# AliBahri94/GM3D

Measured on AMD Instinct MI355X. Metric: point-clouds/sec pretrain step (N=1024,G=64), higher is better.
Workload: dtype bf16

## Files before the change

### gm3d_amd/_capi.py

```python
import ctypes
import os

_HERE = os.path.dirname(os.path.abspath(__file__))
LIB_PATH = os.environ.get("GM3D_HIP_LIB") or os.path.join(_HERE, "lib", "libgm3d_hip.so")

GM3D_OK, GM3D_EINVAL, GM3D_EUNSUPPORTED, GM3D_ELAUNCH = 0, -1, -2, -3
GM3D_F32, GM3D_BF16 = 0, 1

_vp, _i, _f = ctypes.c_void_p, ctypes.c_int, ctypes.c_float

SIGNATURES = {
    "gm3d_abi_version": [],
    "gm3d_strerror": [_i],
    "gm3d_fps": [_vp, _i, _i, _i, _vp, _vp, _vp],
    "gm3d_gather_points": [_vp, _vp, _i, _i, _i, _i, _vp, _vp],
    "gm3d_gather_points_grad": [_vp, _vp, _i, _i, _i, _i, _vp, _vp],
    "gm3d_knn": [_vp, _vp, _i, _i, _i, _i, _vp, _vp, _vp],
    "gm3d_knn_group": [_vp, _vp, _i, _i, _i, _i, _vp, _vp, _vp, _vp],
    "gm3d_chamfer_fwd": [_vp, _vp, _i, _i, _i, _vp, _vp, _vp, _vp, _vp],
    "gm3d_chamfer_bwd": [_vp, _vp, _vp, _vp, _vp, _vp, _i, _i, _i, _vp, _vp, _vp],
    "gm3d_patch_chamfer_loss_fwd": [_vp, ctypes.c_longlong, _vp, _vp, ctypes.c_longlong, _i, _i, _i, _vp, _vp, _vp, _vp, _i, _vp],
    "gm3d_patch_chamfer_loss_bwd": [_vp, ctypes.c_longlong, _vp, _vp, ctypes.c_longlong, _vp, _vp, _vp, _i, _i, _i, _vp, _i, _vp],
    "gm3d_attention_fwd": [_vp, _vp, _vp, _i, _i, _i, _f, _i, _vp],
    "gm3d_attention_qkv_fwd": [_vp, _vp, _vp, _vp, _vp, _i, _i, _i, _i, _f, _i, _vp],
    "gm3d_attention_bwd": [_vp, _vp, _vp, _vp, _vp, _i, _i, _i, _f, _i, _vp],
    "gm3d_ln_plain_partial_rows": [_i],
    "gm3d_ln_plain_fwd": [_vp, _vp, _vp, _f, _vp, _vp, _vp, _i, _i, _i, _vp],
    "gm3d_ln_plain_bwd": [_vp, _vp, _vp, _vp, _vp, _vp, _vp, _i, _i, _i, _vp],
    "gm3d_residual_ln_fwd": [_vp, _vp, _vp, _vp, _i, _vp, _vp, _vp, _f, _vp, _vp, _vp, _vp, _i, _i, _i, _vp],
    "gm3d_residual_ln_bwd": [_vp, _vp, _vp, _vp, _vp, _vp, _vp, _i, _vp, _vp, _vp, _vp, _vp, _i, _i, _i, _vp],
    "gm3d_ln_partial_rows": [_i],
    "gm3d_colsum_finish": [_vp, _i, _i, _i, _vp, _i, _vp],
    "gm3d_colsum_finish_batched": [_vp, _i, ctypes.c_longlong, _i, _i, _i, _vp, _i, _vp],
    "gm3d_bias_gelu_fwd": [_vp, _vp, _vp, _i, _i, _i, _vp],
    "gm3d_bias_gelu_bwd": [_vp, _vp, _vp, _vp, _vp, _i, _i, _i, _vp],
    "gm3d_gelu_partial_rows": [_i],
    "gm3d_embed_partial_rows": [_i, _i, _i],
    "gm3d_moments3": [_vp, _i, _vp, _vp],
    "gm3d_pn_layer1_fwd": [_vp, _vp, _vp, _vp, _i, _i, _i, _vp],
    "gm3d_group_max_fwd": [_vp, _vp, _vp, _vp, _i, _i, _i, _i, _vp],
    "gm3d_group_max_bwd": [_vp, _vp, _vp, _i, _i, _i, _i, _vp],
    "gm3d_bn_bcast_stats": [_vp, _vp, _i, _i, _i, _vp, _i, _vp],
    "gm3d_bn_bcast_apply_relu": [_vp, _vp, _vp, _vp, _vp, _i, _i, _i, _f, _i, _vp],
    "gm3d_bn_bcast_bwd_stats": [_vp, _vp, _vp, _vp, _vp, _vp, _vp, _i, _i, _i, _vp, _f, _i, _vp],
    "gm3d_bn_bcast_bwd_apply": [_vp, _vp, _vp, _vp, _vp, _vp, _vp, _vp, _vp, _vp, _vp, _i, _i, _i, _f, _i, _vp],
    "gm3d_head_fold": [_vp, _vp, _i, _i, _vp, _vp, _vp, _i, _vp],
    "gm3d_head_rowdot": [_vp, _vp, _vp, _i, _i, _vp, _i, _vp],
    "gm3d_head_fold_bwd": [_vp, _vp, _i, _i, _i, _vp, _vp, _vp],
    "gm3d_head_outer": [_vp, _vp, _i, _i, _vp, _i, _vp],
    "gm3d_scale_translate": [_vp, _vp, _f, _f, _f, _i, _i, _vp],
    "gm3d_group_select_maps": [_vp, _i, _i, _i, _i, _vp, _vp, _vp],
    "gm3d_bn_bcast_apply_relu_sel": [_vp, _vp, _vp, _vp, _vp, _vp, _i, _i, _i, _f, _i, _vp],
    "gm3d_bn_bcast_bwd_stats_sel": [_vp, _vp, _vp, _vp, _vp, _vp, _vp, _vp, _i, _i, _i, _vp, _f, _i, _vp],
    "gm3d_bn_bcast_bwd_apply_sel": [_vp, _vp, _vp, _vp, _vp, _vp, _vp, _vp, _vp, _vp, _vp, _vp, _i, _i, _i, _f, _i, _vp],
    "gm3d_lin3_gelu_fwd": [_vp, _vp, _vp, _vp, _i, _i, _i, _vp],
    "gm3d_lin3_gelu_bwd": [_vp, _vp, _vp, _vp, _i, _i, _vp, _i, _vp],
    "gm3d_lin3_finish": [_vp, _i, _i, _vp, _vp, _vp],
    "gm3d_rank_loss": [_vp, _vp, _i, _i, _vp, _vp, _vp],
    "gm3d_rank_loss_tail": [_vp, _i, _vp, _i, _i, _vp, _vp, _vp, _vp, _vp],
    "gm3d_rank_loss_tail_bwd": [_vp, _vp, _vp, _i, _i, _i, _vp, _vp],
    "gm3d_ema_counters": [_vp, _vp, _i, _f, _f, _vp],
    "gm3d_drop_path_scales": [_vp, _vp, _i, _i, _vp, _vp],
    "gm3d_pad_cols": [_vp, ctypes.c_longlong, _i, _i, _vp, _i, _i, _vp],
    "gm3d_patch_chamfer_loss_bwd_full": [_vp, ctypes.c_longlong, _vp, _vp, ctypes.c_longlong, _vp, _vp, _vp, _i, _i, _i, _i, _vp, _i, _vp],
    "gm3d_mask_select_b": [_vp, _vp, _i, _i, _i, _i, _vp, _vp, _vp, _vp, _i, _vp],
    "gm3d_pn1_bwd_finalize": [_vp, _vp, _vp, _vp, _vp, _vp, _vp, _vp, _i, _vp],
    "gm3d_gemm_tn_bf16": [_vp, _vp, _vp, _vp, _i, _i, _i, _i, _i, _i, _vp],
    "gm3d_gemm_tn_bf16_gelu": [_vp, _vp, _vp, _vp, _vp, _i, _i, _i, _i, _i, _i, _i, _vp],
    "gm3d_gemm_tn_bf16_pool": [_vp, _vp, _vp, _vp, _vp, _vp, _i, _i, _i, _i, _i, _i, _i, _i, _vp],
    "gm3d_gemm_tn_bf16_gelu_bwd": [_vp, _vp, _vp, _vp, _vp, _vp, _i, _i, _i, _i, _i, _i, _i, _vp],
    "gm3d_gemm_tn_bf16_res": [_vp, _vp, _vp, _vp, _vp, _i, _vp, _vp, _vp, _vp, _i, _i, _i, _i, _i, _i, _vp],
    "gm3d_gemm_tn_bf16_lna": [_vp, _vp, _vp, _vp, _f, _vp, _vp, _vp, _vp, _vp, _vp, _vp, _i, _i, _i, _i, _i, _i, _i, _vp],
    "gm3d_gemm_tile_rows": [_i],
    "gm3d_gemm_tn_bf16_ring": [_vp, _vp, _vp, _vp, _i, _i, _i, _i, _i, _i, _i, _vp],
    "gm3d_gemm_tn_bf16_ws": [_vp, _vp, _vp, _vp, _i, _i, _i, _i, _i, _i, _vp],
    "gm3d_gemm_tn_bf16_ws_pool": [_vp, _vp, _vp, _vp, _vp, _vp, _i, _i, _i, _i, _i, _i, _i, _i, _vp],
    "gm3d_gemm_ws_supported": [_i, _i, _i],
    "gm3d_gemm_tn_bf16_ws_poolg": [_vp, _vp, _vp, _vp, _vp, _vp, _i, _i, _i, _i, _i, _i, _i, _i, _i, _vp],
    "gm3d_gemm_nt_bf16_sum": [_vp, _vp, _vp, _vp, _vp, _i, _i, _i, _i, _i, _i, _i, ctypes.c_longlong, ctypes.c_longlong, ctypes.c_longlong, _i, _vp],
    "gm3d_gemm_nt_tiles": [_i, _i],
    "gm3d_gemm_nt_bf16_multi": [_i] + [_vp] * 14 + [_vp],
    "gm3d_gemm_tn_bf16_ws_bn_apply": [_vp, _vp, _vp, _vp, _vp, _f, _vp, _i, _i, _i, _i, _i, _i, _i, _vp],
    "gm3d_gemm_tn_bf16_ws_bn_stats": [_vp, _vp, _vp, _vp, _vp, _i, _i, _i, _i, _i, _i, _i, _vp],
    "gm3d_gemm_ws_stats_rows": [_i, _i, _i],
    "gm3d_gemm_tn_bf16_ws_bn_apply_g": [_vp, _vp, _vp, _vp, _vp, _f, _vp, _i, _i, _i, _i, _i, _i, _i, _i, _vp],
    "gm3d_gemm_tn_bf16_ws_bn_stats_g": [_vp, _vp, _vp, _vp, _vp, _i, _i, _i, _i, _i, _i, _i, _i, _vp],
    "gm3d_gemm_tn_bf16_ring96": [_vp, _vp, _vp, _vp, _i, _i, _i, _i, _i, _i, _i, _vp],
    "gm3d_gemm_tn_bf16_dma": [_vp, _vp, _vp, _vp, _i, _i, _i, _i, _i, _i, _i, _vp],
    "gm3d_gemm_tn_bf16_dma_gelu_bwd": [_vp, _vp, _vp, _vp, _vp, _vp, _i, _i, _i, _i, _i, _i, _i, _i, _vp],
    "gm3d_gemm_tn_bf16_dma_gelu": [_vp, _vp, _vp, _vp, _vp, _i, _i, _i, _i, _i, _i, _i, _i, _vp],
    "gm3d_transpose_bf16_batched": [_vp, _vp, _i, _i, _i, ctypes.c_longlong, _vp],
    "gm3d_transpose_bf16_multi": [_i, _vp, _vp, _vp, _vp, _vp, _vp, _vp],
    "gm3d_token_assemble_fwd": [_vp, _vp, _vp, _i, _i, _i, _i, _vp, _vp, _vp, _i, _vp],
    "gm3d_token_assemble_bwd": [_vp, _vp, _vp, _vp, _i, _i, _i, _i, _vp, _vp, _i, _vp],
    "gm3d_sum_few_rows": [_vp, _i, _i, ctypes.c_longlong, _vp, _vp],
    "gm3d_gemm_nt_bf16": [_vp, _vp, _vp, _i, _i, _i, _i, _i, _i, _i, ctypes.c_longlong, ctypes.c_longlong, ctypes.c_longlong, _i,
                          ctypes.c_longlong, _vp],
    "gm3d_gemm_nt_bf16_big": [_vp, _vp, _vp, _i, _i, _i, _i, _i, _i, _i, ctypes.c_longlong, ctypes.c_longlong, ctypes.c_longlong, _i,
                              ctypes.c_longlong, _vp],
    "gm3d_gemm_nt_splits": [_i, _i, _i, _i],
    "gm3d_radius_mask_bits": [_vp, _vp, _f, _i, _i, _vp, _vp],
    "gm3d_radius_mask_bits_m": [_vp, _vp, _i, _f, _i, _i, _vp, _vp],
    "gm3d_attention_masked_fwd": [_vp, _vp, _vp, _vp, _i, _i, _i, _i, _f, _i, _vp],
    "gm3d_attention_masked_bwd": [_vp, _vp, _vp, _vp, _vp, _vp, _i, _i, _i, _i, _f, _i, _vp],
    "gm3d_mask_select": [_vp, _vp, _i, _i, _i, _i, _vp, _vp, _vp, _i, _vp],
    "gm3d_bn_finalize": [_vp, ctypes.c_double, _vp, _vp, _f, _f, _vp, _vp, _vp, _vp, _vp, _vp, _vp, _i, _i, _vp],
    "gm3d_pn1_finalize": [_vp, ctypes.c_double, _vp, _vp, _vp, _vp, _f, _f, _vp, _vp, _vp, _vp, _vp, _vp, _vp, _vp, _vp, _i, _i, _vp],
    "gm3d_flat_partial_rows": [ctypes.c_longlong],
    "gm3d_adamw_ema_flat_step": [_vp, _vp, _vp, _vp, _vp, _vp, _vp, ctypes.c_longlong, ctypes.c_longlong, _vp, _f, _f, _f, _f,
                                 _vp, _f, _vp, _vp, _vp, _vp],
    "gm3d_adamw_ema_flat_step_lrd": [_vp, _vp, _vp, _vp, _vp, _vp, _vp, ctypes.c_longlong, ctypes.c_longlong, _vp, _vp, _f, _f,
                                     _f, _f, _vp, _f, _vp, _vp, _vp, _vp],
    "gm3d_group_scatter_add": [_vp, _vp, _vp, _i, _i, _i, _vp, _i, _vp],
    "gm3d_pn_layer1_bwd_stats": [_vp, _vp, _vp, _vp, _vp, _vp, _vp, _vp, _i, _i, _vp, _i, _vp],
    "gm3d_colsum_finish_f64": [_vp, _i, _i, _i, _vp, _vp],
    "gm3d_colsum_partial": [_vp, _i, _i, _vp, _i, _vp],
    "gm3d_gather_inverse": [_vp, _i, _i, _i, _vp, _vp, _vp],
    "gm3d_gather_rows_bwd": [_vp, _vp, _vp, _vp, _i, _i, _i, _i, _i, _vp],
    "gm3d_add_ln_fwd": [_vp, _vp, _vp, _vp, _i, _vp, _vp, _vp, _f, _vp, _vp, _vp, _vp, _i, _i, _i, _vp],
    "gm3d_add_ln_bwd": [_vp, _vp, _vp, _vp, _vp, _vp, _vp, _i, _vp, _vp, _vp, _i, _i, _i, _i, _vp],
    "gm3d_add_ln_bwd_acc": [_vp, _vp, _vp, _vp, _vp, _vp, _vp, _i, _vp, _vp, _vp, _i, _vp, _i, _i, _i, _i, _vp],
    "gm3d_partition_visible": [_vp, _i, _i, _i, _vp, _vp, _vp, _vp, _vp, _vp, _vp],
    "gm3d_select_rows": [_vp, _vp, _vp, _vp, _i, _i, _i, _i, _i, _vp],
    "gm3d_back_project": [_vp, _vp, _i, _i, _i, _i, _vp, _vp],
    "gm3d_interp3_fwd": [_vp, _vp, _vp, _vp, _vp, _i, _i, _i, _i, _i, _i, _vp],
    "gm3d_gather_rows_bwd_w": [_vp, _i, _i, _i, _vp, _vp, _vp, _vp, _i, _i, _i, _i, _i, _vp],
    "gm3d_where_rows": [_vp, _i, _vp, _vp, _i, _vp, ctypes.c_longlong, _i, _i, _vp],
    "gm3d_take_rows": [_vp, _vp, _vp, _i, _i, _i, _i, _i, _vp],
    "gm3d_colsum_partial_w": [_vp, _vp, _i, _i, _vp, _i, _vp],
    "gm3d_gemm_tn_bf16_dma_pool": [_vp, _vp, _vp, _vp, _vp, _vp, _i, _i, _i, _i, _i, _i, _i, _i, _i, _i, _vp],
    "gm3d_gemm_tn_bf16_dmaw": [_vp, _vp, _vp, _vp, _i, _i, _i, _i, _i, _i, _i, _i, _vp],
    "gm3d_vote_sample": [_vp, _vp, _vp, _vp, _vp, _i, _i, _i, _i, _i, _vp, _vp],
    "gm3d_cls_tail_vote": [_vp, _i, _i, _i, _i] + [_vp] * 14 + [_i, _f, _vp, _vp, _vp, _vp, _vp, _i, _vp],
    "gm3d_cls_tail_fwd": [_vp, _i, _i, _i, _i] + [_vp] * 10 + [_i] + [_vp] * 6 + [_f, _f, _i] + [_vp] * 8 + [_i, _vp],
    "gm3d_cls_tail_bwd": [_i, _i, _i, _i] + [_vp] * 7 + [_i, _i] + [_vp] * 21 + [_i, _vp],
    "gm3d_cls_tail_vote_pool": [_vp, _i, _i, _i, _i, _i] + [_vp] * 14 + [_i, _f, _vp, _vp, _vp, _vp, _vp, _vp, _i, _vp],
    "gm3d_svm_gram": [_vp, _i, _i, _vp, _vp],
    "gm3d_svm_smo": [_vp, _i, _i, _vp, ctypes.c_double, ctypes.c_double, ctypes.c_longlong, _vp, _vp, _vp, _vp, _vp],
    "gm3d_svm_weights": [_vp, _i, _i, _i, _vp, _vp, _vp, _vp],
    "gm3d_svm_predict": [_vp, _i, _i, _i, _vp, _vp, _vp, _vp, _vp, _vp],
}


class Gm3dError(RuntimeError):
    pass


def _load():
    if not os.path.exists(LIB_PATH):
        raise ImportError(
            "gm3d_amd: %s not found. Build it with `python -m gm3d_amd.build` "
            "(hipcc, --offload-arch=gfx950). There is no CPU fallback." % LIB_PATH)
    lib = ctypes.CDLL(LIB_PATH)
    for name, argtypes in SIGNATURES.items():
        fn = getattr(lib, name)
        fn.argtypes = argtypes
        fn.restype = ctypes.c_char_p if name == "gm3d_strerror" else ctypes.c_int
    return lib


lib = _load()


def check(rc, what):
    if rc != GM3D_OK:
        raise Gm3dError("%s failed: %s (code %d)" % (what, lib.gm3d_strerror(rc).decode(), rc))
```

### gm3d_amd/csrc/gemm_dma.hip

```cpp
#include "mfma.hpp"

namespace gm3d {

constexpr int DBK = 64;

template <int WMI, int EPI, int NJ>
__global__ __launch_bounds__(256, 2) void gemm_tn_dma_kernel(const bf16_t* __restrict__ A, const bf16_t* __restrict__ W,
                                                             const float* __restrict__ bias, bf16_t* __restrict__ C, int M, int N, int K,
                                                             int lda, int ldw, int ldc, int tiles_n, int total_tiles,
                                                             bf16_t* __restrict__ G, int ldg, const bf16_t* __restrict__ Fpre,
                                                             int ldfp, float* __restrict__ colpart, uint8_t* __restrict__ ARG,
                                                             int bias_after_pool) {
    extern __shared__ __attribute__((aligned(16))) unsigned char dsm[];
    constexpr int BM = 64 * WMI, DBN = 64 * NJ;
    constexpr int STAGE = (BM + DBN) * 128;
    constexpr int PA = BM / 8, PIECES = (PA + DBN / 8) / 4;
    const int tid = threadIdx.x, lane = tid & 63, w = __builtin_amdgcn_readfirstlane(tid >> 6);
    const int r = lane & 31, hh = lane >> 5;
    const int logical = xcd_tile(blockIdx.x, gridDim.x);
    if (logical >= total_tiles) return;
    const int tile_m = logical / tiles_n, tile_n = logical - tile_m * tiles_n;
    const int m0 = tile_m * BM, n0 = tile_n * DBN;
    const int wm = (w >> 1) * 32 * WMI, wn = (w & 1) * 32 * NJ;
    const unsigned lds0 = lds_addr(dsm);

    const int prow = lane >> 3, pslot = lane & 7;
    const bf16_t* src[PIECES];
#pragma unroll
    for (int i = 0; i < PIECES; ++i) {
        const int p = w + 4 * i;
        if (p < PA) {
            const int row = 8 * p + prow;
            const int am = m0 + row < M ? m0 + row : M - 1;
            src[i] = A + (size_t)am * lda + ((pslot ^ swz(row)) << 3);
        } else {
            const int row = 8 * (p - PA) + prow;
            src[i] = W + (size_t)(n0 + row) * ldw + ((pslot ^ swz(row)) << 3);
        }
    }
#define GM3D_DMA_STAGE(ST)                                                                          \
    {                                                                                               \
        const unsigned base = lds0 + ((ST) & 1) * STAGE;                                            \
        _Pragma("unroll") for (int i = 0; i < PIECES; ++i)                                          \
            glds16(src[i] + (size_t)(ST) * DBK, base + 1024 * (w + 4 * i));                         \
    }
    f32x16 acc[WMI][NJ];
#pragma unroll
    for (int i = 0; i < WMI; ++i)
#pragma unroll
        for (int j = 0; j < NJ; ++j)
#pragma unroll
            for (int g = 0; g < 16; ++g) acc[i][j][g] = 0.f;

    const int KT = K / DBK;
    GM3D_DMA_STAGE(0)
    for (int kt = 0; kt < KT; ++kt) {
        asm volatile("s_waitcnt vmcnt(0)" ::: "memory");
        __builtin_amdgcn_s_barrier();
        if (kt + 1 < KT) GM3D_DMA_STAGE(kt + 1)
        const unsigned char* as = dsm + (kt & 1) * STAGE;
        const unsigned char* ws = as + BM * 128;
#pragma unroll
        for (int s = 0; s < 4; ++s) {
            bf16x8 fa[WMI];
#pragma unroll
            for (int i = 0; i < WMI; ++i) fa[i] = *reinterpret_cast<const bf16x8*>(as + swz_off(wm + 32 * i + r, 2 * s + hh));
#pragma unroll
            for (int j = 0; j < NJ; ++j) {
                const bf16x8 fw = *reinterpret_cast<const bf16x8*>(ws + swz_off(wn + 32 * j + r, 2 * s + hh));
#pragma unroll
                for (int i = 0; i < WMI; ++i) acc[i][j] = mfma_bf16(fw, fa[i], acc[i][j]);
            }
        }
    }
#undef GM3D_DMA_STAGE
    __syncthreads();
#pragma unroll
    for (int i = 0; i < WMI; ++i)
#pragma unroll
        for (int j = 0; j < NJ; ++j) {
            const int row = wm + 32 * i + r, col = wn + 32 * j;
            unsigned char* img = dsm + (col >> 6) * (BM * 128);
            const int cbase = (col & 63) >> 3;
#pragma unroll
            for (int q = 0; q < 4; ++q) {
                float v[4] = {acc[i][j][4 * q], acc[i][j][4 * q + 1], acc[i][j][4 * q + 2], acc[i][j][4 * q + 3]};
                if ((EPI == 0 || (EPI == 3 && !bias_after_pool)) && bias) {
                    const float4 b = *reinterpret_cast<const float4*>(bias + n0 + col + 8 * q + 4 * hh);
                    v[0] += b.x; v[1] += b.y; v[2] += b.z; v[3] += b.w;
                }
                bf16x4 pk;
#pragma unroll
                for (int e = 0; e < 4; ++e) pk[e] = (bf16_t)v[e];
                *reinterpret_cast<bf16x4*>(img + swz_off(row, cbase + q) + 8 * hh) = pk;
            }
        }
    __syncthreads();
    if (EPI == 3) {
        constexpr int CH = DBN / 8;
        if (tid < (BM / 32) * CH) {
            const int g = tid / CH, chunk = tid - g * CH;
            if (m0 + 32 * g < M) {
                const unsigned char* img = dsm + (chunk >> 3) * (BM * 128);
                float best[8];
                int bk[8];
#pragma unroll
                for (int e = 0; e < 8; ++e) { best[e] = -INFINITY; bk[e] = 0; }
#pragma unroll 8
                for (int k = 0; k < 32; ++k) {
                    const bf16x8 f = *reinterpret_cast<const bf16x8*>(img + swz_off(32 * g + k, chunk & 7));
#pragma unroll
                    for (int e = 0; e < 8; ++e) {
                        const float v = (float)f[e];
                        if (v > best[e]) { best[e] = v; bk[e] = k; }
                    }
                }
                const int n = n0 + 8 * chunk;
                if (bias_after_pool && bias) {
                    float bv[8];
                    V8<float>::load(bias + n, bv);
#pragma unroll
                    for (int e = 0; e < 8; ++e) best[e] += bv[e];
                }
                const size_t o = (size_t)((m0 + 32 * g) >> 5) * ldg + n;
                V8<bf16_t>::store(G + o, best);
                unsigned long long pk = 0;
#pragma unroll
                for (int e = 0; e < 8; ++e) pk |= (unsigned long long)(bk[e] & 0xff) << (8 * e);
                *reinterpret_cast<unsigned long long*>(ARG + o) = pk;
            }
        }
        if (!C) return;
    }
    float csum[NJ][8];
#pragma unroll
    for (int t = 0; t < NJ; ++t)
#pragma unroll
        for (int e = 0; e < 8; ++e) csum[t][e] = 0.f;
#pragma unroll
    for (int i = 0; i < 2 * NJ * WMI; ++i) {
        const int c = tid + 256 * i;
        const int t = i / (2 * WMI), row = (c - t * (BM * 8)) >> 3, ch = tid & 7;
        if (m0 + row < M) {
            const uint4 raw = *reinterpret_cast<const uint4*>(dsm + t * (BM * 128) + swz_off(row, ch));
            const int n = n0 + 64 * t + 8 * ch;
            if (EPI == 0 || EPI == 3) {
                *reinterpret_cast<uint4*>(C + (size_t)(m0 + row) * ldc + n) = raw;
            } else {
                const bf16x8 f = *reinterpret_cast<const bf16x8*>(&raw);
                float bv[8], v[8];
                V8<float>::load(bias + n, bv);
                if (EPI == 1) {
                    if (C) *reinterpret_cast<uint4*>(C + (size_t)(m0 + row) * ldc + n) = raw;
#pragma unroll
                    for (int e = 0; e < 8; ++e) v[e] = gelu_f<bf16_t>((float)f[e] + bv[e]);
                    V8<bf16_t>::store(G + (size_t)(m0 + row) * ldg + n, v);
                } else {
                    float fv[8];
                    V8<bf16_t>::load(Fpre + (size_t)(m0 + row) * ldfp + n, fv);
#pragma unroll
                    for (int e = 0; e < 8; ++e) {
                        v[e] = (float)f[e] * gelu_grad_f<bf16_t>(fv[e] + bv[e]);
                        csum[t][e] += v[e];
                    }
                    V8<bf16_t>::store(C + (size_t)(m0 + row) * ldc + n, v);
                }
            }
        }
    }
    if (EPI == 2) {
        __syncthreads();
        float* cs = reinterpret_cast<float*>(dsm);
#pragma unroll
        for (int t = 0; t < NJ; ++t)
#pragma unroll
            for (int e = 0; e < 8; ++e) cs[(tid >> 3) * DBN + 64 * t + 8 * (tid & 7) + e] = csum[t][e];
        __syncthreads();
        if (tid < DBN) {
            float s = 0.f;
#pragma unroll
            for (int k = 0; k < 32; ++k) s += cs[k * DBN + tid];
            colpart[(size_t)tile_m * N + n0 + tid] = s;
        }
    }
}

}

static int dma_launch(const void* A, const void* W, const float* bias, void* C, void* G, int M, int N, int K, int lda, int ldw, int ldc,
                      int ldg, int bm, gm3d_stream_t stream, const void* Fpre = nullptr, int ldfp = 0, float* colpart = nullptr,
                      int bn = 192, uint8_t* ARG = nullptr, int bias_after_pool = 0) {
    using namespace gm3d;
    if (!A || !W || (!C && !G) || M < 0 || N < 1 || K < 1) return GM3D_EINVAL;
    if ((G || Fpre) && !bias && !ARG) return GM3D_EINVAL;
    if (ARG && (!G || Fpre || M % 32 || ldg % 8 || ((size_t)ARG & 7) || (bn != 128 && bn != 192))) return GM3D_EINVAL;
    if (Fpre && (!C || !colpart || G || ldfp % 8 || ldfp < N || ((size_t)Fpre & 15))) return GM3D_EINVAL;
    if (bn != 128 && bn != 192 && bn != 256) return GM3D_EUNSUPPORTED;
    if ((G || Fpre) && !ARG && bn != 192) return GM3D_EUNSUPPORTED;
    if (N % bn || K % DBK || lda % 8 || ldw % 8 || lda < K || ldw < K || (C && (ldc % 8 || ldc < N)) || (G && (ldg % 8 || ldg < N)))
        return GM3D_EUNSUPPORTED;
    if ((((size_t)A | (size_t)W | (size_t)C | (size_t)G) & 15) || (bm != 64 && bm != 128)) return GM3D_EUNSUPPORTED;
    if (M == 0) return GM3D_OK;
    const int tiles_m = (M + bm - 1) / bm, tiles_n = N / bn;
    if ((long long)tiles_m * tiles_n > 0x7ffffff0LL) return GM3D_EUNSUPPORTED;
    const int total = tiles_m * tiles_n, grid = (total + 7) / 8 * 8;
    const size_t lds = (size_t)2 * (bm + bn) * 128;
#define GM3D_DMA(WMI, EPI, NJ)                                                                                            \
    launch_lds<gemm_tn_dma_kernel<WMI, EPI, NJ>>(dim3(grid), dim3(256), lds, stream, (const bf16_t*)A, (const bf16_t*)W, bias,  \
                                                 (bf16_t*)C, M, N, K, lda, ldw, ldc, tiles_n, total, (bf16_t*)G, ldg,          \
                                                 (const bf16_t*)Fpre, ldfp, colpart, ARG, bias_after_pool)
    if (ARG) {
        if (bn == 128) return bm == 64 ? GM3D_DMA(1, 3, 2) : GM3D_DMA(2, 3, 2);
        return bm == 64 ? GM3D_DMA(1, 3, 3) : GM3D_DMA(2, 3, 3);
    }
    if (Fpre) return bm == 64 ? GM3D_DMA(1, 2, 3) : GM3D_DMA(2, 2, 3);
    if (G) return bm == 64 ? GM3D_DMA(1, 1, 3) : GM3D_DMA(2, 1, 3);
    if (bn == 192) return bm == 64 ? GM3D_DMA(1, 0, 3) : GM3D_DMA(2, 0, 3);
    if (bn == 128) return bm == 64 ? GM3D_DMA(1, 0, 2) : GM3D_DMA(2, 0, 2);
    return bm == 64 ? GM3D_DMA(1, 0, 4) : GM3D_DMA(2, 0, 4);
#undef GM3D_DMA
}

extern "C" int gm3d_gemm_tn_bf16_dma(const void* A, const void* W, const float* bias, void* C, int M, int N, int K, int lda, int ldw,
                                     int ldc, int bm, gm3d_stream_t stream) {
    if (!C) return GM3D_EINVAL;
    return dma_launch(A, W, bias, C, nullptr, M, N, K, lda, ldw, ldc, 0, bm, stream);
}

extern "C" int gm3d_gemm_tn_bf16_dmaw(const void* A, const void* W, const float* bias, void* C, int M, int N, int K, int lda, int ldw,
                                      int ldc, int bm, int bn, gm3d_stream_t stream) {
    if (!C) return GM3D_EINVAL;
    return dma_launch(A, W, bias, C, nullptr, M, N, K, lda, ldw, ldc, 0, bm, stream, nullptr, 0, nullptr, bn);
}

extern "C" int gm3d_gemm_tn_bf16_dma_pool(const void* A, const void* W, const float* bias, void* C, void* P, uint8_t* arg, int M, int N,
                                          int K, int lda, int ldw, int ldc, int ldp, int bias_after_pool, int bm, int bn,
                                          gm3d_stream_t stream) {
    if (!P || !arg) return GM3D_EINVAL;
    return dma_launch(A, W, bias, C, P, M, N, K, lda, ldw, ldc, ldp, bm, stream, nullptr, 0, nullptr, bn, arg, bias_after_pool);
}

extern "C" int gm3d_gemm_tn_bf16_dma_gelu(const void* A, const void* W, const float* bias, void* F, void* G, int M, int N, int K,
                                          int lda, int ldw, int ldf, int ldg, int bm, gm3d_stream_t stream) {
    if (!G || !bias) return GM3D_EINVAL;
    return dma_launch(A, W, bias, F, G, M, N, K, lda, ldw, ldf, ldg, bm, stream);
}

extern "C" int gm3d_gemm_tn_bf16_dma_gelu_bwd(const void* dO, const void* Wt, const void* F, const float* bias, void* dF, float* colpart,
                                              int M, int N, int K, int lda, int ldw, int ldf, int lddf, int bm, gm3d_stream_t stream) {
    if (!F || !bias || !dF || !colpart) return GM3D_EINVAL;
    return dma_launch(dO, Wt, bias, dF, nullptr, M, N, K, lda, ldw, lddf, 0, bm, stream, F, ldf, colpart);
}
```

### gm3d_amd/csrc/gemm_ring.hip

```cpp
#include "mfma.hpp"

namespace gm3d {

constexpr int RBN = 128, RBK = 64, RNBUF = 4, RCP = 132;

template <int WMI, bool RES, int DEPTH>
__global__ __launch_bounds__(256) void gemm_tn_ring_kernel(const bf16_t* __restrict__ A, const bf16_t* __restrict__ W,
                                                           const float* __restrict__ bias, bf16_t* __restrict__ C, int M, int N, int K,
                                                           int lda, int ldw, int ldc, int tiles_n, int total_tiles,
                                                           const float* __restrict__ res, const float* __restrict__ rowscale,
                                                           int rows_per_sample, const bf16_t* __restrict__ add, float* __restrict__ U,
                                                           float* __restrict__ stats, bf16_t* __restrict__ U16) {
    extern __shared__ __attribute__((aligned(16))) unsigned char rsm[];
    constexpr int BM = 64 * WMI;
    constexpr int STAGE = (BM + RBN) * 128;
    constexpr int PA = BM / 8, PIECES = (PA + 16) / 4;
    const int tid = threadIdx.x, lane = tid & 63, w = __builtin_amdgcn_readfirstlane(tid >> 6);
    const int r = lane & 31, hh = lane >> 5;
    const int logical = xcd_tile(blockIdx.x, gridDim.x);
    if (logical >= total_tiles) return;
    const int tile_m = logical / tiles_n, tile_n = logical - tile_m * tiles_n;
    const int m0 = tile_m * BM, n0 = tile_n * RBN;
    const int wm = (w >> 1) * 32 * WMI, wn = (w & 1) * 64;
    const unsigned lds0 = lds_addr(rsm);

    const int prow = lane >> 3, pslot = lane & 7;
    const bf16_t* src[PIECES];
#pragma unroll
    for (int i = 0; i < PIECES; ++i) {
        const int p = w + 4 * i;
        if (p < PA) {
            const int row = 8 * p + prow;
            const int am = m0 + row < M ? m0 + row : M - 1;
            src[i] = A + (size_t)am * lda + ((pslot ^ swz(row)) << 3);
        } else {
            const int row = 8 * (p - PA) + prow;
            const int wn_ = n0 + row < N ? n0 + row : N - 1;
            src[i] = W + (size_t)wn_ * ldw + ((pslot ^ swz(row)) << 3);
        }
    }
    constexpr int NBUF = DEPTH + 2;
#define GM3D_RING_STAGE(ST)                                                                          \
    {                                                                                                \
        const unsigned base = lds0 + ((ST) % NBUF) * STAGE;                                          \
        _Pragma("unroll") for (int i = 0; i < PIECES; ++i)                                           \
            glds16(src[i] + (size_t)(ST) * RBK, base + 1024 * (w + 4 * i));                          \
    }

    f32x16 acc[WMI][2];
#pragma unroll
    for (int i = 0; i < WMI; ++i)
#pragma unroll
        for (int j = 0; j < 2; ++j)
#pragma unroll
            for (int g = 0; g < 16; ++g) acc[i][j][g] = 0.f;

    const int KT = K / RBK;
#pragma unroll
    for (int d = 0; d < DEPTH; ++d)
        if (d < KT) GM3D_RING_STAGE(d)
    for (int kt = 0; kt < KT; ++kt) {
        if (kt + DEPTH < KT) {
            GM3D_RING_STAGE(kt + DEPTH)
            asm volatile("s_waitcnt vmcnt(%0)" ::"n"(DEPTH * PIECES) : "memory");
        } else {
            const int rem = KT - 1 - kt;
            if (DEPTH > 3 && rem == 3) asm volatile("s_waitcnt vmcnt(%0)" ::"n"(3 * PIECES) : "memory");
            else if (DEPTH > 2 && rem == 2) asm volatile("s_waitcnt vmcnt(%0)" ::"n"(2 * PIECES) : "memory");
            else if (rem == 1) asm volatile("s_waitcnt vmcnt(%0)" ::"n"(PIECES) : "memory");
            else asm volatile("s_waitcnt vmcnt(0)" ::: "memory");
        }
        __builtin_amdgcn_s_barrier();
        const unsigned char* as = rsm + (kt % NBUF) * STAGE;
        const unsigned char* ws = as + BM * 128;
        bf16x8 fa[4][WMI], fw[4][2];
#pragma unroll
        for (int s = 0; s < 4; ++s) {
#pragma unroll
            for (int i = 0; i < WMI; ++i) fa[s][i] = *reinterpret_cast<const bf16x8*>(as + swz_off(wm + 32 * i + r, 2 * s + hh));
#pragma unroll
            for (int j = 0; j < 2; ++j) fw[s][j] = *reinterpret_cast<const bf16x8*>(ws + swz_off(wn + 32 * j + r, 2 * s + hh));
        }
#pragma unroll
        for (int s = 0; s < 4; ++s)
#pragma unroll
            for (int i = 0; i < WMI; ++i)
#pragma unroll
                for (int j = 0; j < 2; ++j) acc[i][j] = mfma_bf16(fw[s][j], fa[s][i], acc[i][j]);
    }
#undef GM3D_RING_STAGE
    __syncthreads();
    float* cs = reinterpret_cast<float*>(rsm);
#pragma unroll
    for (int i = 0; i < WMI; ++i)
#pragma unroll
        for (int j = 0; j < 2; ++j)
#pragma unroll
            for (int q = 0; q < 4; ++q) {
                const int m = wm + 32 * i + r, n = wn + 32 * j + 8 * q + 4 * hh;
                *reinterpret_cast<float4*>(cs + m * RCP + n) =
                    make_float4(acc[i][j][4 * q], acc[i][j][4 * q + 1], acc[i][j][4 * q + 2], acc[i][j][4 * q + 3]);
            }
    __syncthreads();
    if (RES) {
#pragma unroll
        for (int i = 0; i < 4 * WMI; ++i) {
            const int c = tid + 256 * i;
            const int row = c >> 4, nc = (c & 15) * 8;
            const bool valid = m0 + row < M;
            const int gr = valid ? m0 + row : M - 1;
            float v[8], rv[8];
            const float4 x = *reinterpret_cast<const float4*>(cs + row * RCP + nc), y = *reinterpret_cast<const float4*>(cs + row * RCP + nc + 4);
            v[0] = x.x; v[1] = x.y; v[2] = x.z; v[3] = x.w; v[4] = y.x; v[5] = y.y; v[6] = y.z; v[7] = y.w;
#pragma unroll
            for (int e = 0; e < 8; ++e) v[e] = (float)(bf16_t)v[e];
            if (bias) {
                const float4 b0 = *reinterpret_cast<const float4*>(bias + n0 + nc), b1 = *reinterpret_cast<const float4*>(bias + n0 + nc + 4);
                v[0] += b0.x; v[1] += b0.y; v[2] += b0.z; v[3] += b0.w; v[4] += b1.x; v[5] += b1.y; v[6] += b1.z; v[7] += b1.w;
            }
            const float rs = rowscale ? rowscale[gr / rows_per_sample] : 1.0f;
            V8<float>::load(res + (size_t)gr * N + n0 + nc, rv);
#pragma unroll
            for (int e = 0; e < 8; ++e) v[e] = rv[e] + rs * v[e];
            if (add) {
                float av[8];
                V8<bf16_t>::load(add + (size_t)gr * N + n0 + nc, av);
#pragma unroll
                for (int e = 0; e < 8; ++e) v[e] += av[e];
            }
            if (valid) {
                V8<float>::store(U + (size_t)gr * N + n0 + nc, v);
                V8<bf16_t>::store(U16 + (size_t)gr * N + n0 + nc, v);
            }
            float sm = 0.f;
#pragma unroll
            for (int e = 0; e < 8; ++e) sm += v[e];
            sm += __shfl_xor(sm, 1); sm += __shfl_xor(sm, 2); sm += __shfl_xor(sm, 4); sm += __shfl_xor(sm, 8);
            const float mu = sm * (1.0f / 128.0f);
            float q = 0.f;
#pragma unroll
            for (int e = 0; e < 8; ++e) { const float d = v[e] - mu; q += d * d; }
            q += __shfl_xor(q, 1); q += __shfl_xor(q, 2); q += __shfl_xor(q, 4); q += __shfl_xor(q, 8);
            if (valid && (c & 15) == 0) {
                float* sp = stats + ((size_t)tile_n * M + gr) * 2;
                sp[0] = mu;
                sp[1] = q;
            }
        }
        return;
    }
#pragma unroll
    for (int i = 0; i < 4 * WMI; ++i) {
        const int c = tid + 256 * i;
        const int row = c >> 4, nc = (c & 15) * 8;
        if (m0 + row < M && n0 + nc < N) {
            float v[8];
            const float4 x = *reinterpret_cast<const float4*>(cs + row * RCP + nc), y = *reinterpret_cast<const float4*>(cs + row * RCP + nc + 4);
            v[0] = x.x; v[1] = x.y; v[2] = x.z; v[3] = x.w; v[4] = y.x; v[5] = y.y; v[6] = y.z; v[7] = y.w;
            if (bias) {
                const float4 b0 = *reinterpret_cast<const float4*>(bias + n0 + nc), b1 = *reinterpret_cast<const float4*>(bias + n0 + nc + 4);
                v[0] += b0.x; v[1] += b0.y; v[2] += b0.z; v[3] += b0.w; v[4] += b1.x; v[5] += b1.y; v[6] += b1.z; v[7] += b1.w;
            }
            V8<bf16_t>::store(C + (size_t)(m0 + row) * ldc + n0 + nc, v);
        }
    }
}

constexpr int R96 = 96, RCP96 = 100;

template <int WMI>
__global__ __launch_bounds__(192) void gemm_tn_ring96_kernel(const bf16_t* __restrict__ A, const bf16_t* __restrict__ W,
                                                             const float* __restrict__ bias, bf16_t* __restrict__ C, int M, int N, int K,
                                                             int lda, int ldw, int ldc, int tiles_n, int total_tiles) {
    extern __shared__ __attribute__((aligned(16))) unsigned char rsm[];
    constexpr int BM = 64 * WMI, NMT = 2 * WMI;
    constexpr int STAGE = (BM + R96) * 128;
    constexpr int PA = BM / 8, NP = PA + 12;
    constexpr int PMAX = (NP + 2) / 3;
    const int tid = threadIdx.x, lane = tid & 63, w = __builtin_amdgcn_readfirstlane(tid >> 6);
    const int r = lane & 31, hh = lane >> 5;
    const int logical = xcd_tile(blockIdx.x, gridDim.x);
    if (logical >= total_tiles) return;
    const int tile_m = logical / tiles_n, tile_n = logical - tile_m * tiles_n;
    const int m0 = tile_m * BM, n0 = tile_n * R96;
    const unsigned lds0 = lds_addr(rsm);
    const int mine = (NP - w + 2) / 3;

    const int prow = lane >> 3, pslot = lane & 7;
    const bf16_t* src[PMAX];
#pragma unroll
    for (int i = 0; i < PMAX; ++i) {
        const int p = w + 3 * i < NP ? w + 3 * i : w;
        if (p < PA) {
            const int row = 8 * p + prow;
            const int am = m0 + row < M ? m0 + row : M - 1;
            src[i] = A + (size_t)am * lda + ((pslot ^ swz(row)) << 3);
        } else {
            const int row = 8 * (p - PA) + prow;
            src[i] = W + (size_t)(n0 + row) * ldw + ((pslot ^ swz(row)) << 3);
        }
    }
#define GM3D_R96_STAGE(ST)                                                                           \
    {                                                                                                \
        const unsigned base = lds0 + ((ST) % RNBUF) * STAGE;                                         \
        _Pragma("unroll") for (int i = 0; i < PMAX; ++i)                                             \
            if (i < mine) glds16(src[i] + (size_t)(ST) * RBK, base + 1024 * (w + 3 * i));            \
    }
    f32x16 acc[NMT];
#pragma unroll
    for (int i = 0; i < NMT; ++i)
#pragma unroll
        for (int g = 0; g < 16; ++g) acc[i][g] = 0.f;

    const int KT = K / RBK;
    GM3D_R96_STAGE(0)
    if (KT > 1) GM3D_R96_STAGE(1)
    for (int kt = 0; kt < KT; ++kt) {
        if (kt + 2 < KT) {
            GM3D_R96_STAGE(kt + 2)
            if (mine == PMAX) asm volatile("s_waitcnt vmcnt(%0)" ::"n"(2 * PMAX) : "memory");
            else asm volatile("s_waitcnt vmcnt(%0)" ::"n"(2 * (PMAX - 1)) : "memory");
        } else if (kt + 1 < KT) {
            if (mine == PMAX) asm volatile("s_waitcnt vmcnt(%0)" ::"n"(PMAX) : "memory");
            else asm volatile("s_waitcnt vmcnt(%0)" ::"n"(PMAX - 1) : "memory");
        } else {
            asm volatile("s_waitcnt vmcnt(0)" ::: "memory");
        }
        __builtin_amdgcn_s_barrier();
        const unsigned char* as = rsm + (kt % RNBUF) * STAGE;
        const unsigned char* ws = as + BM * 128;
        bf16x8 fa[4][NMT], fw[4];
#pragma unroll
        for (int s = 0; s < 4; ++s) {
#pragma unroll
            for (int i = 0; i < NMT; ++i) fa[s][i] = *reinterpret_cast<const bf16x8*>(as + swz_off(32 * i + r, 2 * s + hh));
            fw[s] = *reinterpret_cast<const bf16x8*>(ws + swz_off(32 * w + r, 2 * s + hh));
        }
#pragma unroll
        for (int s = 0; s < 4; ++s)
#pragma unroll
            for (int i = 0; i < NMT; ++i) acc[i] = mfma_bf16(fw[s], fa[s][i], acc[i]);
    }
#undef GM3D_R96_STAGE
    __syncthreads();
    float* cs = reinterpret_cast<float*>(rsm);
#pragma unroll
    for (int i = 0; i < NMT; ++i)
#pragma unroll
        for (int q = 0; q < 4; ++q) {
            const int m = 32 * i + r, n = 32 * w + 8 * q + 4 * hh;
            *reinterpret_cast<float4*>(cs + m * RCP96 + n) = make_float4(acc[i][4 * q], acc[i][4 * q + 1], acc[i][4 * q + 2], acc[i][4 * q + 3]);
        }
    __syncthreads();
#pragma unroll
    for (int i = 0; i < BM * 12 / 192; ++i) {
        const int c = tid + 192 * i;
        const int row = c / 12, nc = (c - row * 12) * 8;
        if (m0 + row < M) {
            float v[8];
            const float4 x = *reinterpret_cast<const float4*>(cs + row * RCP96 + nc), y = *reinterpret_cast<const float4*>(cs + row * RCP96 + nc + 4);
            v[0] = x.x; v[1] = x.y; v[2] = x.z; v[3] = x.w; v[4] = y.x; v[5] = y.y; v[6] = y.z; v[7] = y.w;
            if (bias) {
                const float4 b0 = *reinterpret_cast<const float4*>(bias + n0 + nc), b1 = *reinterpret_cast<const float4*>(bias + n0 + nc + 4);
                v[0] += b0.x; v[1] += b0.y; v[2] += b0.z; v[3] += b0.w; v[4] += b1.x; v[5] += b1.y; v[6] += b1.z; v[7] += b1.w;
            }
            V8<bf16_t>::store(C + (size_t)(m0 + row) * ldc + n0 + nc, v);
        }
    }
}

}

static constexpr int RING_DEPTH = 2;

static int ring_launch(const void* A, const void* W, const float* bias, void* C, int M, int N, int K, int lda, int ldw, int ldc, int bm,
                       gm3d_stream_t stream, const float* res, const float* rowscale, int rows_per_sample, const void* add, float* U,
                       float* stats, void* U16) {
    using namespace gm3d;
    if (!A || !W || (!C && !U) || M < 0 || N < 1 || K < 1) return GM3D_EINVAL;
    if (N % 8 || (U && N % RBN) || K % RBK || lda % 8 || ldw % 8 || lda < K || ldw < K || (C && (ldc % 8 || ldc < N)))
        return GM3D_EUNSUPPORTED;
    if ((((size_t)A | (size_t)W) & 15) || (bm != 64 && bm != 128)) return GM3D_EUNSUPPORTED;
    if (M == 0) return GM3D_OK;
    const int tiles_m = (M + bm - 1) / bm, tiles_n = (N + RBN - 1) / RBN;
    if ((long long)tiles_m * tiles_n > 0x7ffffff0LL) return GM3D_EUNSUPPORTED;
    const int total = tiles_m * tiles_n, grid = (total + 7) / 8 * 8;
    const size_t lds = (size_t)(RING_DEPTH + 2) * (bm + RBN) * 128;
#define GM3D_RING(WMI, RES)                                                                                                     \
    launch_lds<gemm_tn_ring_kernel<WMI, RES, RING_DEPTH>>(dim3(grid), dim3(256), lds, stream, (const bf16_t*)A, (const bf16_t*)W, \
                                                          bias, (bf16_t*)C, M, N, K, lda, ldw, ldc, tiles_n, total, res, rowscale, \
                                                          rows_per_sample, (const bf16_t*)add, U, stats, (bf16_t*)U16)
    if (U) return bm == 64 ? GM3D_RING(1, true) : GM3D_RING(2, true);
    return bm == 64 ? GM3D_RING(1, false) : GM3D_RING(2, false);
#undef GM3D_RING
}

extern "C" int gm3d_gemm_tn_bf16_ring(const void* A, const void* W, const float* bias, void* C, int M, int N, int K, int lda, int ldw,
                                      int ldc, int bm, gm3d_stream_t stream) {
    if (!C) return GM3D_EINVAL;
    return ring_launch(A, W, bias, C, M, N, K, lda, ldw, ldc, bm, stream, nullptr, nullptr, 1, nullptr, nullptr, nullptr, nullptr);
}

extern "C" int gm3d_gemm_tn_bf16_ring96(const void* A, const void* W, const float* bias, void* C, int M, int N, int K, int lda, int ldw,
                                        int ldc, int bm, gm3d_stream_t stream) {
    using namespace gm3d;
    if (!A || !W || !C || M < 0 || N < 1 || K < 1) return GM3D_EINVAL;
    if (N % R96 || K % RBK || lda % 8 || ldw % 8 || lda < K || ldw < K || ldc % 8 || ldc < N) return GM3D_EUNSUPPORTED;
    if ((((size_t)A | (size_t)W | (size_t)C) & 15) || (bm != 64 && bm != 128)) return GM3D_EUNSUPPORTED;
    if (M == 0) return GM3D_OK;
    const int tiles_m = (M + bm - 1) / bm, tiles_n = N / R96;
    if ((long long)tiles_m * tiles_n > 0x7ffffff0LL) return GM3D_EUNSUPPORTED;
    const int total = tiles_m * tiles_n, grid = (total + 7) / 8 * 8;
    const size_t lds = (size_t)RNBUF * (bm + R96) * 128;
    if (bm == 64)
        return launch_lds<gemm_tn_ring96_kernel<1>>(dim3(grid), dim3(192), lds, stream, (const bf16_t*)A, (const bf16_t*)W, bias,
                                                    (bf16_t*)C, M, N, K, lda, ldw, ldc, tiles_n, total);
    return launch_lds<gemm_tn_ring96_kernel<2>>(dim3(grid), dim3(192), lds, stream, (const bf16_t*)A, (const bf16_t*)W, bias, (bf16_t*)C,
                                                M, N, K, lda, ldw, ldc, tiles_n, total);
}

extern "C" int gm3d_gemm_tn_bf16_res(const void* A, const void* W, const float* bias, const float* res, const float* rowscale,
                                     int rows_per_sample, const void* add, float* U, void* U16, float* stats, int M, int N, int K,
                                     int lda, int ldw, int bm, gm3d_stream_t stream) {
    if (!res || !U || !U16 || !stats || N != 384 || (rowscale && rows_per_sample < 1)) return GM3D_EINVAL;
    return ring_launch(A, W, bias, nullptr, M, N, K, lda, ldw, 0, bm, stream, res, rowscale, rows_per_sample, add, U, stats, U16);
}
```

### gm3d_amd/csrc/mfma.hpp

```cpp
#pragma once
#include "common.hpp"

namespace gm3d {

typedef __bf16 bf16x8 __attribute__((ext_vector_type(8)));
typedef __bf16 bf16x4 __attribute__((ext_vector_type(4)));
typedef float f32x16 __attribute__((ext_vector_type(16)));
typedef __attribute__((address_space(3))) bf16x4 lds_bf16x4;

__device__ __forceinline__ f32x16 mfma_bf16(bf16x8 a, bf16x8 b, f32x16 c) {
    return __builtin_amdgcn_mfma_f32_32x32x16_bf16(a, b, c, 0, 0, 0);
}

__device__ __forceinline__ int crow(int g, int hh) { return (g & 3) + 8 * (g >> 2) + 4 * hh; }

__device__ __forceinline__ bf16x8 zero8() {
    bf16x8 z;
#pragma unroll
    for (int j = 0; j < 8; ++j) z[j] = (bf16_t)0.0f;
    return z;
}
__device__ __forceinline__ f32x16 zero16() {
    f32x16 z;
#pragma unroll
    for (int g = 0; g < 16; ++g) z[g] = 0.f;
    return z;
}
__device__ __forceinline__ bf16x8 cvt8(const f32x16& x, int s, float mul) {
    bf16x8 v;
#pragma unroll
    for (int j = 0; j < 8; ++j) v[j] = (bf16_t)(x[8 * s + j] * mul);
    return v;
}

__device__ __forceinline__ int swz(int row) { return (((row >> 1) & 1) << 2) | (((row >> 2) & 1) << 1) | ((row >> 3) & 1); }
__device__ __forceinline__ int swz_off(int row, int ch) { return row * 128 + ((ch ^ swz(row)) << 4); }

__device__ __forceinline__ unsigned lds_addr(const unsigned char* p) {
    return (unsigned)(size_t)(__attribute__((address_space(3))) const unsigned char*)p;
}

__device__ __forceinline__ void glds16(const void* gsrc, unsigned dst) {
    unsigned keep;
    asm volatile("s_mov_b32 %0, m0\n\ts_mov_b32 m0, %2\n\ts_nop 0\n\tglobal_load_lds_dwordx4 %1, off\n\ts_mov_b32 m0, %0"
                 : "=&s"(keep)
                 : "v"(gsrc), "s"(dst)
                 : "memory");
}

template <class I> __device__ __forceinline__ int xcd_tile(I block, I grid) {
    const int per_xcd = grid >> 3;
    return (block & 7) * per_xcd + (block >> 3);
}

}
```

### gm3d_amd/fused.py

```python
import weakref

import contextlib

import torch

from ._capi import lib
from . import gemm
from . import streams as _streams
from .ops import _launch, _ptr, _stream, _DT

LNC = 384


class _WeightCache:

    def __init__(self):
        self._c = {}
        self._pinned = {}
        self._groups = []

    def pin(self, model, dtype=torch.bfloat16, static=False):
        src = [p for p in model.parameters() if p.dim() >= 2 and p.dtype == torch.float32 and p.is_cuda
               and not self._is_pinned(p)]
        if not src:
            return
        dst = [torch.empty_like(p, dtype=dtype) for p in src]
        for p, d in zip(src, dst):
            self._pinned[p.data_ptr()] = (d, weakref.ref(p))
        if static:
            with torch.no_grad():
                torch._foreach_copy_(dst, [p.detach() for p in src])
            return
        self._groups.append(([p.detach() for p in src], dst))
        with torch.no_grad():
            torch._foreach_copy_(dst, self._groups[-1][0])

    def pin_view(self, p, shadow):
        self._pinned[p.data_ptr()] = (shadow, weakref.ref(p))
        gemm.forget_transposes()

    def _is_pinned(self, p):
        hit = self._pinned.get(p.data_ptr())
        return hit is not None and hit[1]() is p

    def refresh(self):
        with torch.no_grad():
            for src, dst in self._groups:
                torch._foreach_copy_(dst, src)

    def get(self, w, dtype):
        if w.dtype == dtype:
            return w
        hit = self._pinned.get(w.data_ptr())
        if hit is not None and hit[1]() is w and hit[0].dtype == dtype:
            return hit[0]
        base = w._base
        if base is not None and base.dtype == w.dtype:
            hit = self._pinned.get(base.data_ptr())
            if hit is not None and hit[1]() is base and hit[0].dtype == dtype and hit[0].numel() == base.numel():
                return torch.as_strided(hit[0], w.size(), w.stride(), hit[0].storage_offset() + w.storage_offset() - base.storage_offset())
        if torch.cuda.is_current_stream_capturing():
            return w.detach().to(dtype)
        key = (w.data_ptr(), dtype, tuple(w.shape))
        hit = self._c.get(key)
        if hit is not None and hit[0] == w._version and hit[2]() is w:
            if w.is_cuda:
                cur = torch.cuda.current_stream(w.device)
                if hit[3] != cur.cuda_stream:
                    cur.wait_event(hit[4])
                    hit[1].record_stream(cur)
            return hit[1]
        with torch.no_grad():
            c = w.detach().to(dtype)
        if len(self._c) > 4096:
            self._c.clear()
        stream_id, done = None, None
        if w.is_cuda:
            cur = torch.cuda.current_stream(w.device)
            stream_id, done = cur.cuda_stream, torch.cuda.Event()
            done.record(cur)
        self._c[key] = (w._version, c, weakref.ref(w), stream_id, done)
        return c


weight_cache = _WeightCache()


def residual_ln_fwd(res, y, bias, rowscale, rows_per_sample, add, gamma, beta, eps, adt, R, want_res=True, h=None):
    dev = gamma.device
    out_res = torch.empty(R, LNC, dtype=torch.float32, device=dev) if want_res else None
    if h is None:
        h = torch.empty(R, LNC, dtype=adt, device=dev)
    mean = torch.empty(R, dtype=torch.float32, device=dev)
    rstd = torch.empty(R, dtype=torch.float32, device=dev)
    _launch("gm3d_residual_ln_fwd", {"R": R, "dtype": str(adt)}, lib.gm3d_residual_ln_fwd, _ptr(res), _ptr(y), _ptr(bias),
            _ptr(rowscale), int(rows_per_sample), _ptr(add), _ptr(gamma), _ptr(beta), float(eps), _ptr(out_res), _ptr(h),
            _ptr(mean), _ptr(rstd), R, LNC, _DT[adt], _stream())
    return out_res, h, mean, rstd


def residual_ln_bwd(dh, gin, x, mean, rstd, gamma, rowscale, rows_per_sample, acc, want_dy, adt, R, dy=None, partial=None,
                    acc_out=None):
    dev = gamma.device
    dx = torch.empty(R, LNC, dtype=torch.float32, device=dev)
    if dy is None and want_dy:
        dy = torch.empty(R, LNC, dtype=adt, device=dev)
    nrows = lib.gm3d_ln_partial_rows(R)
    defer = partial is not None
    if partial is None:
        partial = torch.empty(nrows, 3 * LNC, dtype=torch.float32, device=dev)
    _launch("gm3d_residual_ln_bwd", {"R": R, "dtype": str(adt)}, lib.gm3d_residual_ln_bwd, _ptr(dh), _ptr(gin), _ptr(x),
            _ptr(mean), _ptr(rstd), _ptr(gamma), _ptr(rowscale), int(rows_per_sample), _ptr(dx), _ptr(dy), _ptr(acc),
            _ptr(acc_out), _ptr(partial), R, LNC, _DT[adt], _stream())
    if defer:
        return dx, dy, None
    sums = torch.empty(3, LNC, dtype=torch.float32, device=dev)
    _launch("gm3d_colsum_finish", {"rows": nrows, "cols": 3 * LNC}, lib.gm3d_colsum_finish, _ptr(partial), nrows, 3 * LNC,
            3 * LNC, _ptr(sums), 0, _stream())
    return dx, dy, sums


def bias_gelu_fwd(f, bias, adt, g=None):
    R, C = f.shape
    if g is None:
        g = torch.empty_like(f)
    _launch("gm3d_bias_gelu_fwd", {"R": R, "C": C, "dtype": str(adt)}, lib.gm3d_bias_gelu_fwd, _ptr(f), _ptr(bias), _ptr(g),
            R, C, _DT[adt], _stream())
    return g


def bias_gelu_bwd(dg, f, bias, adt, df=None, partial=None):
    R, C = f.shape
    if df is None:
        df = torch.empty_like(f)
    nrows = lib.gm3d_gelu_partial_rows(R)
    defer = partial is not None
    if partial is None:
        partial = torch.empty(nrows, C, dtype=torch.float32, device=f.device)
    _launch("gm3d_bias_gelu_bwd", {"R": R, "C": C, "dtype": str(adt)}, lib.gm3d_bias_gelu_bwd, _ptr(dg), _ptr(f), _ptr(bias),
            _ptr(df), _ptr(partial), R, C, _DT[adt], _stream())
    if defer:
        return df, None
    db = torch.empty(C, dtype=torch.float32, device=f.device)
    _launch("gm3d_colsum_finish", {"rows": nrows, "cols": C}, lib.gm3d_colsum_finish, _ptr(partial), nrows, C, C, _ptr(db), 0,
            _stream())
    return df, db


def finish_batched(partial, out):
    J, rows, cols = partial.shape
    _launch("gm3d_colsum_finish_batched", {"rows": J * rows, "cols": cols}, lib.gm3d_colsum_finish_batched, _ptr(partial), J,
            rows * cols, rows, cols, cols, _ptr(out), cols, _stream())
    return out


def _attention_fwd(qkv, B, T, H, scale, out=None):
    if out is None:
        out = torch.empty(B * T, H * 64, dtype=qkv.dtype, device=qkv.device)
    lse = torch.empty(B, H, T, dtype=torch.float32, device=qkv.device)
    if T > 128:
        _launch("gm3d_attention_masked_fwd", {"B": B, "T": T, "H": H, "HD": 64, "dtype": str(qkv.dtype)}, lib.gm3d_attention_masked_fwd,
                _ptr(qkv), None, _ptr(out), _ptr(lse), B, T, H, 64, float(scale), _DT[qkv.dtype], _stream())
        return out, lse
    _launch("gm3d_attention_fwd", {"B": B, "T": T, "H": H, "dtype": str(qkv.dtype)}, lib.gm3d_attention_fwd, _ptr(qkv),
            _ptr(out), _ptr(lse), B, T, H, float(scale), _DT[qkv.dtype], _stream())
    return out, lse


def _attention_qkv_fwd(h, wqkv, B, T, H, scale, out=None, want_qkv=False, want_lse=False):
    C = h.shape[1]
    if out is None:
        out = torch.empty(B * T, C, dtype=h.dtype, device=h.device)
    lse = torch.empty(B, H, T, dtype=torch.float32, device=h.device) if want_lse else None
    qkv = torch.empty(B * T, 3 * C, dtype=h.dtype, device=h.device) if want_qkv else None
    _launch("gm3d_attention_qkv_fwd", {"B": B, "T": T, "H": H, "C": C, "dtype": str(h.dtype)}, lib.gm3d_attention_qkv_fwd, _ptr(h),
            _ptr(wqkv), _ptr(out), _ptr(lse) if want_lse else None, _ptr(qkv) if want_qkv else None, B, T, H, C, float(scale),
            _DT[h.dtype], _stream())
    return out, lse, qkv


def attention_qkv_supported(h, wqkv, T, H):
    return (h.is_cuda and h.dtype == torch.bfloat16 and wqkv.dtype == torch.bfloat16 and T <= 64 and h.shape[1] == 384 == H * 64
            and h.is_contiguous() and wqkv.is_contiguous() and tuple(wqkv.shape) == (1152, 384)
            and h.data_ptr() % 16 == 0 and wqkv.data_ptr() % 16 == 0)


def _attention_bwd(qkv, out, dout, lse, B, T, H, scale, dqkv=None):
    if dqkv is None:
        dqkv = torch.empty_like(qkv)
    if T > 128:
        _launch("gm3d_attention_masked_bwd", {"B": B, "T": T, "H": H, "HD": 64, "dtype": str(qkv.dtype)}, lib.gm3d_attention_masked_bwd,
                _ptr(qkv), None, _ptr(out), _ptr(dout), _ptr(lse), _ptr(dqkv), B, T, H, 64, float(scale), _DT[qkv.dtype], _stream())
        return dqkv
    _launch("gm3d_attention_bwd", {"B": B, "T": T, "H": H, "dtype": str(qkv.dtype)}, lib.gm3d_attention_bwd, _ptr(qkv),
            _ptr(out), _ptr(dout), _ptr(lse), _ptr(dqkv), B, T, H, float(scale), _DT[qkv.dtype], _stream())
    return dqkv


def _wgrad_batched(dy, x, out=None):
    nblk, R, N = dy.shape
    K = x.shape[2]
    if gemm.wgrad_supported(dy, x) and (out is None or (out.stride(2) == 1 and out.stride(1) == K and out.stride(0) == N * K)):
        return gemm.wgrad_nt(dy, x, out)
    S = WGRAD_ROW_SPLIT
    if S == 0:
        S, tiles = 1, nblk * max(N // 128, 1) * max(K // 128, 1)
        while tiles * S < 512 and S < 8 and R % (2 * S) == 0 and R // (2 * S) >= 512:
            S *= 2
    elif nblk > 4 or R // S < 1024:
        S = 1
    if S > 1 and R % S == 0 and dy.is_contiguous() and x.is_contiguous():
        part = _wgrad_batched_plain(dy.view(nblk * S, R // S, N), x.view(nblk * S, R // S, K))
        if out is None:
            out = torch.empty(nblk, N, K, dtype=torch.float32, device=dy.device)
        if SUM_FEW_ROWS:
            _launch("gm3d_sum_few_rows", {"rows": nblk * S, "cols": N * K}, lib.gm3d_sum_few_rows, _ptr(part), nblk, S, N * K,
                    _ptr(out), _stream())
        else:
            _launch("gm3d_colsum_finish_batched", {"rows": nblk * S, "cols": N * K}, lib.gm3d_colsum_finish_batched, _ptr(part), nblk,
                    S * N * K, S, N * K, N * K, _ptr(out), N * K, _stream())
        return out
    return _wgrad_batched_plain(dy, x, out)


SUM_FEW_ROWS = True
WGRAD_ROW_SPLIT = 4


_BMM_OUT_OK = [True]


def _wgrad_batched_plain(dy, x, out=None):
    if dy.dtype == torch.float32:
        return torch.bmm(dy.transpose(1, 2), x) if out is None else torch.bmm(dy.transpose(1, 2), x, out=out)
    if out is not None and _BMM_OUT_OK[0]:
        try:
            return torch.bmm(dy.transpose(1, 2), x, out_dtype=torch.float32, out=out)
        except (TypeError, RuntimeError):
            _BMM_OUT_OK[0] = False
    try:
        r = torch.bmm(dy.transpose(1, 2), x, out_dtype=torch.float32)
    except TypeError:
        r = torch.bmm(dy.transpose(1, 2), x).float()
    return r if out is None else out.copy_(r)


WGRAD_MIN_BLOCKS = 5
_ASYNC_WGRAD = {"stream": None, "used": False, "min_blocks": 5, "deferred": []}


def _wgrad_many(reqs):
    if gemm.MULTI_WGRAD and len(reqs) > 1 and all(gemm.wgrad_multi_ok(dy, x, out) for dy, x, out in reqs):
        if len(reqs) <= 16:
            return gemm.wgrad_nt_multi(reqs)
        res = []
        per = -(-len(reqs) // -(-len(reqs) // 16))
        for i in range(0, len(reqs), per):
            chunk = reqs[i:i + per]
            res += gemm.wgrad_nt_multi(chunk) if len(chunk) > 1 else [_wgrad_batched(*chunk[0])]
        return res
    return [_wgrad_batched(dy, x, out) for dy, x, out in reqs]


def defer_wgrad(dy, x, w=None):
    reg = _ASYNC_WGRAD
    if (reg["stream"] is not None and gemm.MULTI_WGRAD and (DEFER_HEAD_WGRAD or reg.get("defer_heads")) and w is not None and w.is_leaf and w.grad is None
            and dy.dim() == 2
            and dy.is_contiguous() and x.is_contiguous()):
        from .optim import grad_slots, ENABLE_DIRECT_WGRAD
        slot = grad_slots.get(w) if ENABLE_DIRECT_WGRAD else None
        if slot is not None and slot.is_contiguous() and slot.numel() == dy.shape[1] * x.shape[1]:
            out = slot.view(1, dy.shape[1], x.shape[1])
            if gemm.wgrad_multi_ok(dy.unsqueeze(0), x.unsqueeze(0), out):
                reg["deferred"].append(((dy, x), [(dy.unsqueeze(0), x.unsqueeze(0), out)]))
                return out[0]
    from .embed import splitk_wgrad
    return splitk_wgrad(dy, x)


DEFER_HEAD_WGRAD = False


def _run_deferred(reg, own=()):
    jobs, reg["deferred"] = reg["deferred"], []
    cur = torch.cuda.current_stream()
    reqs = []
    for tensors, rq in jobs:
        for t in tensors:
            t.record_stream(cur)
        reqs += rq
    res = _wgrad_many(reqs + list(own)) if (reqs or own) else []
    return res[len(reqs):]

_wgrad_streams = {}
ASYNC_WGRAD = True


class async_wgrad:

    def __init__(self, device, min_blocks=None, defer_heads=False):
        self.dev, self.min_blocks = torch.device(device), (WGRAD_MIN_BLOCKS if min_blocks is None else min_blocks)
        self.defer_heads = bool(defer_heads)

    def __enter__(self):
        if ASYNC_WGRAD and self.dev.type == "cuda":
            key = (self.dev.type, self.dev.index)
            if key not in _wgrad_streams:
                _wgrad_streams[key] = torch.cuda.Stream(device=self.dev)
            _ASYNC_WGRAD.update(stream=_wgrad_streams[key], used=False, min_blocks=self.min_blocks, defer_heads=self.defer_heads)
            if self.defer_heads:
                gemm.prepare_transposes()
        return self

    def __exit__(self, *exc):
        reg = _ASYNC_WGRAD
        ws, used = reg["stream"], reg["used"]
        if reg.get("defer_heads"):
            gemm.drop_transposes()
        reg.update(stream=None, used=False, defer_heads=False)
        if reg["deferred"]:
            if exc[0] is None:
                _run_deferred(reg)
            reg["deferred"] = []
        if ws is not None and used:
            _streams.join(ws)
        return False


DIRECT_INPUT_GRADS = True
FUSE_QKV_ATTENTION = True
PER_BLOCK = 11


def block_params(block):
    return [block.norm1.weight, block.norm1.bias, block.attn.qkv.weight, block.attn.proj.weight, block.attn.proj.bias,
            block.norm2.weight, block.norm2.bias, block.mlp.fc1.weight, block.mlp.fc1.bias, block.mlp.fc2.weight,
            block.mlp.fc2.bias]


def _mm(x, w):
    return gemm.mm(x, w)


class TransformerStackFn(torch.autograd.Function):

    @staticmethod
    def forward(ctx, x, pos, meta, final_w, final_b, *params):
        with torch.autocast("cuda", enabled=False):
            return TransformerStackFn._forward(ctx, x, pos, meta, final_w, final_b, *params)

    @staticmethod
    def _forward(ctx, x, pos, meta, final_w, final_b, *params):
        g = TransformerStackFn._forward_gen(ctx, x, pos, meta, final_w, final_b, *params)
        while True:
            try:
                next(g)
            except StopIteration as done:
                return done.value

    @staticmethod
    def _forward_gen(ctx, x, pos, meta, final_w, final_b, *params):
        B, T, C = x.shape
        assert C == LNC and len(params) % PER_BLOCK == 0
        nblk = len(params) // PER_BLOCK
        adt, H, scale, eps = meta["adt"], meta["num_heads"], meta["scale"], meta["eps"]
        R = B * T
        posa = pos.reshape(R, C).to(adt).contiguous()
        need = meta["grad"] and any(ctx.needs_input_grad)
        y = bias = rs = None
        if x.dtype == adt and adt != torch.float32:
            res, y = None, x.reshape(R, C).contiguous()
        else:
            res = x.reshape(R, C).float().contiguous()
        saved = []
        dev = x.device
        if need:
            H1 = torch.empty(nblk, R, C, dtype=adt, device=dev)
            A = torch.empty(nblk, R, C, dtype=adt, device=dev)
            H2 = torch.empty(nblk, R, C, dtype=adt, device=dev)
            GG = torch.empty(nblk, R, 4 * C, dtype=adt, device=dev)
        fuse_ln = (gemm.ENABLED and gemm.FUSE_LN and gemm.FUSE_GELU and adt == torch.bfloat16 and x.is_cuda
                   and all(gemm.supported(posa, weight_cache.get(params[i * PER_BLOCK + k], adt)) or k == 9
                           for i in range(nblk) for k in (2, 3, 7)))
        st1 = None
        for i in range(nblk):
            ln1w, ln1b, wqkv, wproj, bproj, ln2w, ln2b, w1, b1, w2, b2 = params[i * PER_BLOCK:(i + 1) * PER_BLOCK]
            dp1, dp2 = meta["dp"][i]
            if fuse_ln:
                if i == 0:
                    u, h1, m1, r1 = residual_ln_fwd(res, y, bias, rs, T, posa, ln1w, ln1b, eps, adt, R, h=H1[i] if need else None)
                    yield
                    qkv = _mm(h1, weight_cache.get(wqkv, adt))
                else:
                    qkv, m1, r1 = gemm.linear_lna(u16, st1, ln1w, ln1b, eps, weight_cache.get(wqkv, adt), None,
                                                  h_out=H1[i] if need else None, want_stats=need)
                yield
                a, lse = _attention_fwd(qkv, B, T, H, scale, out=A[i] if need else None)
                yield
                x1, x16, st2 = gemm.linear_res(a, weight_cache.get(wproj, adt), bproj, u, dp1, T, None)
                yield
                W1 = weight_cache.get(w1, adt)
                f, g, m2, r2 = gemm.linear_lna(x16, st2, ln2w, ln2b, eps, W1, b1, gelu=True,
                                               f_out=torch.empty(R, W1.shape[0], dtype=adt, device=dev) if need else None,
                                               g_out=GG[i] if need else None, h_out=H2[i] if need else None, want_stats=need)
                yield
                if need:
                    saved += [u, m1, r1, qkv, lse, x1, m2, r2, f]
                if i + 1 < nblk:
                    u, u16, st1 = gemm.linear_res(g, weight_cache.get(w2, adt), b2, x1, dp2, T, posa)
                else:
                    o = _mm(g, weight_cache.get(w2, adt))
                    res, y, bias, rs = x1, o, b2, dp2
                yield
                continue
            u, h1, m1, r1 = residual_ln_fwd(res, y, bias, rs, T, posa, ln1w, ln1b, eps, adt, R, h=H1[i] if need else None)
            yield
            Wq = weight_cache.get(wqkv, adt)
            if FUSE_QKV_ATTENTION and T > 32 and attention_qkv_supported(h1, Wq, T, H):
                a, lse, qkv = _attention_qkv_fwd(h1, Wq, B, T, H, scale, out=A[i] if need else None, want_qkv=need, want_lse=need)
            else:
                qkv = _mm(h1, Wq)
                yield
                a, lse = _attention_fwd(qkv, B, T, H, scale, out=A[i] if need else None)
            yield
            p = _mm(a, weight_cache.get(wproj, adt))
            yield
            x1, h2, m2, r2 = residual_ln_fwd(u, p, bproj, dp1, T, None, ln2w, ln2b, eps, adt, R, h=H2[i] if need else None)
            yield
            W1 = weight_cache.get(w1, adt)
            if gemm.FUSE_GELU and gemm.supported(h2, W1):
                fo = torch.empty(R, W1.shape[0], dtype=adt, device=dev) if need else None
                if gemm.dma_supported(h2, W1):
                    f, g = gemm.linear_gelu_dma(h2, W1, b1, f_out=fo, g_out=GG[i] if need else None, bm=gemm.dma_bm(R))
                else:
                    f, g = gemm.linear_gelu(h2, W1, b1, f_out=fo, g_out=GG[i] if need else None)
            else:
                f = h2 @ W1.t()
                yield
                g = bias_gelu_fwd(f, b1, adt, g=GG[i] if need else None)
            yield
            o = _mm(g, weight_cache.get(w2, adt))
            yield
            if need:
                saved += [u, m1, r1, qkv, lse, x1, m2, r2, f]
            res, y, bias, rs = x1, o, b2, dp2
        xf, hout, mf, rf = residual_ln_fwd(res, y, bias, rs, T, None, final_w, final_b, meta["final_eps"], adt, R,
                                           want_res=need, h=meta.get("hout"))
        if need:
            ctx.save_for_backward(final_w, xf, mf, rf, H1, A, H2, GG, *params, *saved)
        ctx.meta, ctx.shape, ctx.nblk = meta, (B, T, C), nblk
        ctx.in_dtypes = (x.dtype, pos.dtype)
        return hout.view(B, T, C)

    @staticmethod
    def backward(ctx, dout):
        with torch.autocast("cuda", enabled=False):
            return TransformerStackFn._backward(ctx, dout)

    @staticmethod
    def _backward(ctx, dout):
        meta, (B, T, C), nblk = ctx.meta, ctx.shape, ctx.nblk
        adt, H, scale = meta["adt"], meta["num_heads"], meta["scale"]
        R = B * T
        tens = ctx.saved_tensors
        final_w, xf, mf, rf, H1, A, H2, GG = tens[:8]
        params = tens[8:8 + nblk * PER_BLOCK]
        saved = tens[8 + nblk * PER_BLOCK:]
        grads = [None] * (nblk * PER_BLOCK)
        dev = dout.device
        dh = dout.reshape(R, C).to(adt).contiguous()
        DO = torch.empty(nblk, R, C, dtype=adt, device=dev)
        DF = torch.empty(nblk, R, 4 * C, dtype=adt, device=dev)
        DP = torch.empty(nblk, R, C, dtype=adt, device=dev)
        DQ = torch.empty(nblk, R, 3 * C, dtype=adt, device=dev)
        PLN = torch.empty(2 * nblk + 1, lib.gm3d_ln_partial_rows(R), 3 * C, dtype=torch.float32, device=dev)
        SLN = torch.empty(2 * nblk + 1, 3, C, dtype=torch.float32, device=dev)
        w2s = [weight_cache.get(params[i * PER_BLOCK + 9], adt) for i in range(nblk)]
        fuse_mlp_bwd = gemm.ENABLED and gemm.FUSE_GELU_BWD and adt == torch.bfloat16 and dh.is_cuda
        if fuse_mlp_bwd:
            W2T, WPT, W1T, WQT = gemm.stacked_transposes(
                [w2s] + [[weight_cache.get(params[i * PER_BLOCK + k], adt) for i in range(nblk)] for k in (3, 7, 2)])
        dma_bwd = fuse_mlp_bwd and gemm.dma_supported(dh.reshape(R, C), W2T[0])
        bm_bwd = gemm.dma_bm(R)
        PGL = torch.empty(nblk, ((R + bm_bwd - 1) // bm_bwd if dma_bwd else gemm.tile_rows(R)) if fuse_mlp_bwd
                          else lib.gm3d_gelu_partial_rows(R), 4 * C, dtype=torch.float32, device=dev)
        SGL = torch.empty(nblk, 4 * C, dtype=torch.float32, device=dev)
        dp2_last = meta["dp"][nblk - 1][1]
        G, d_o, _ = residual_ln_bwd(dh, None, xf, mf, rf, final_w, dp2_last, T, None, True, adt, R, dy=DO[nblk - 1],
                                    partial=PLN[2 * nblk])
        g_final_w, g_final_b, db2 = SLN[2 * nblk, 0], SLN[2 * nblk, 1], SLN[2 * nblk, 2]
        dpos = torch.zeros(R, C, dtype=torch.float32, device=dev) if nblk == 1 else None
        for i in range(nblk - 1, -1, -1):
            ln1w, ln1b, wqkv, wproj, bproj, ln2w, ln2b, w1, b1, w2, b2 = params[i * PER_BLOCK:(i + 1) * PER_BLOCK]
            u, m1, r1, qkv, lse, x1, m2, r2, f = saved[i * 9:(i + 1) * 9]
            dp1 = meta["dp"][i][0]
            dp2_prev = meta["dp"][i - 1][1] if i > 0 else None
            gi = grads[i * PER_BLOCK:(i + 1) * PER_BLOCK]
            gi[10] = db2
            if fuse_mlp_bwd:
                df = (gemm.linear_gelu_bwd_dma(d_o, W2T[i], f, b1, DF[i], PGL[i], bm=bm_bwd) if dma_bwd
                      else gemm.linear_gelu_bwd(d_o, W2T[i], f, b1, DF[i], PGL[i]))
            else:
                dg = d_o @ weight_cache.get(w2, adt)
                df, _ = bias_gelu_bwd(dg, f, b1, adt, df=DF[i], partial=PGL[i])
            gi[8] = SGL[i]
            dh2 = gemm.mm(df, W1T[i]) if fuse_mlp_bwd else df @ weight_cache.get(w1, adt)
            dx1, d_p, _ = residual_ln_bwd(dh2, G, x1, m2, r2, ln2w, dp1, T, None, True, adt, R, dy=DP[i],
                                          partial=PLN[2 * i + 1])
            gi[5], gi[6], gi[4] = SLN[2 * i + 1, 0], SLN[2 * i + 1, 1], SLN[2 * i + 1, 2]
            da = gemm.mm(d_p, WPT[i]) if fuse_mlp_bwd else d_p @ weight_cache.get(wproj, adt)
            dqkv = _attention_bwd(qkv, A[i], da, lse, B, T, H, scale, dqkv=DQ[i])
            dh1 = gemm.mm(dqkv, WQT[i]) if fuse_mlp_bwd else dqkv @ weight_cache.get(wqkv, adt)
            last = DIRECT_INPUT_GRADS and i == 0 and nblk > 1 and adt != torch.float32 and ctx.in_dtypes == (adt, adt)
            if last:
                dx_a = torch.empty(R, C, dtype=adt, device=dev)
                dpos_a = torch.empty(R, C, dtype=adt, device=dev)
                G, _, _ = residual_ln_bwd(dh1, dx1, u, m1, r1, ln1w, None, T, dpos, True, adt, R, dy=dx_a, partial=PLN[0],
                                          acc_out=dpos_a)
            else:
                G, d_o, _ = residual_ln_bwd(dh1, dx1, u, m1, r1, ln1w, dp2_prev, T, dpos, i > 0, adt, R,
                                            dy=DO[i - 1] if i > 0 else None, partial=PLN[2 * i])
            if dpos is None:
                dpos = G
            gi[0], gi[1] = SLN[2 * i, 0], SLN[2 * i, 1]
            db2 = SLN[2 * i, 2]
            grads[i * PER_BLOCK:(i + 1) * PER_BLOCK] = gi
        finish_batched(PLN, SLN.view(2 * nblk + 1, 3 * C))
        finish_batched(PGL, SGL)
        from .optim import grad_slots
        def slot(k):
            ps = [params[i * PER_BLOCK + k] for i in range(nblk)]
            return grad_slots.stacked(ps) if dev.type == "cuda" and all(p.grad is None for p in ps) else None
        reg = _ASYNC_WGRAD
        fresh = dev.type == "cuda" and all(params[i * PER_BLOCK + k].grad is None for i in range(nblk) for k in (9, 7, 3, 2))
        ws = reg["stream"] if fresh else None
        slots = [slot(k) for k in (9, 7, 3, 2)] if fresh else [None] * 4
        jobs = [(DO, GG), (DF, H2), (DP, A), (DQ, H1)]
        own = [(dy_, x_, sl) for (dy_, x_), sl in zip(jobs, slots)]
        if ws is not None and nblk < reg["min_blocks"] and all(sl is not None for sl in slots):
            reg["deferred"].append(((DO, GG, DF, H2, DP, A, DQ, H1), own))
            gw2, gw1, gwp, gwq = slots
        else:
            if ws is not None and nblk >= reg["min_blocks"]:
                _streams.fork(ws, who="fused.TransformerStackFn.backward: weight-gradient stream (async_wgrad region)")
                reg["used"] = True
                for t in (DO, GG, DF, H2, DP, A, DQ, H1):
                    t.record_stream(ws)
            else:
                ws = None
            with (torch.cuda.stream(ws) if ws is not None else contextlib.nullcontext()):
                gw2, gw1, gwp, gwq = _run_deferred(reg, own) if ws is not None else _wgrad_many(own)
        for i in range(nblk):
            grads[i * PER_BLOCK + 9], grads[i * PER_BLOCK + 7] = gw2[i], gw1[i]
            grads[i * PER_BLOCK + 3], grads[i * PER_BLOCK + 2] = gwp[i], gwq[i]
        if last:
            return (dx_a.view(B, T, C), dpos_a.view(B, T, C), None, g_final_w, g_final_b) + tuple(grads)
        dx = G.view(B, T, C).to(ctx.in_dtypes[0])
        return (dx, dpos.view(B, T, C).to(ctx.in_dtypes[1]), None, g_final_w, g_final_b) + tuple(grads)


def run_stack(blocks, final_norm, x, pos, training):
    from . import models_mae_learn_loss as M
    blocks = list(blocks)
    adt = torch.bfloat16 if (torch.is_autocast_enabled() and torch.get_autocast_dtype("cuda") == torch.bfloat16) \
        or x.dtype == torch.bfloat16 else torch.float32
    B = x.shape[0]
    probs = []
    for b in blocks:
        p = getattr(b.drop_path, "drop_prob", 0.0)
        probs += [p, p]
    scales = M.drop_path_scales(B, probs, training, x.device)
    dp = [(scales[2 * i], scales[2 * i + 1]) for i in range(len(blocks))]
    meta = {"num_heads": blocks[0].attn.num_heads, "scale": blocks[0].attn.scale, "eps": blocks[0].norm1.eps,
            "final_eps": final_norm.eps, "adt": adt, "dp": dp, "grad": torch.is_grad_enabled()}
    params = []
    for b in blocks:
        params += block_params(b)
    ns = NOGRAD_SPLIT
    if (ns > 1 and x.is_cuda and not training and B % ns == 0 and B // ns >= 16
            and not (torch.is_grad_enabled() and (x.requires_grad or params[0].requires_grad))):
        main = torch.cuda.current_stream()
        h = B // ns
        x, pos = x.contiguous(), pos.contiguous()
        outs = [None] * ns
        streams = [main] + [_split_stream(x.device, j) for j in range(1, ns)]
        for side in streams[1:]:
            _streams.fork(side, main, who="fused.run_stack: parallel inference chain (NOGRAD_SPLIT)")
            x.record_stream(side)
            pos.record_stream(side)
        if LOCKSTEP:
            T_, C_ = x.shape[1], x.shape[2]
            out = torch.empty(B, T_, C_, dtype=adt, device=x.device)
            for side in streams[1:]:
                out.record_stream(side)
            with torch.autocast("cuda", enabled=False), torch.no_grad():
                gens = [TransformerStackFn._forward_gen(_NoCtx(), x[j * h:(j + 1) * h], pos[j * h:(j + 1) * h],
                                                        dict(meta, hout=out[j * h:(j + 1) * h].view(h * T_, C_)), final_norm.weight,
                                                        final_norm.bias, *params) for j in range(ns)]
                live = ns
                while live:
                    for j in range(ns):
                        if gens[j] is None:
                            continue
                        with torch.cuda.stream(streams[j]):
                            try:
                                next(gens[j])
                            except StopIteration as done:
                                outs[j], gens[j] = done.value, None
                                live -= 1
        else:
            for j in range(1, ns):
                with torch.cuda.stream(streams[j]):
                    outs[j] = TransformerStackFn.apply(x[j * h:(j + 1) * h], pos[j * h:(j + 1) * h], meta, final_norm.weight,
                                                       final_norm.bias, *params)
            outs[0] = TransformerStackFn.apply(x[:h], pos[:h], meta, final_norm.weight, final_norm.bias, *params)
        for j in range(1, ns):
            _streams.join(streams[j], main)
            outs[j].record_stream(main)
        return out if LOCKSTEP else torch.cat(outs, dim=0)
    return TransformerStackFn.apply(x, pos, meta, final_norm.weight, final_norm.bias, *params)


class _NoCtx:
    needs_input_grad = ()

    def save_for_backward(self, *a):
        pass


LOCKSTEP = True
NOGRAD_SPLIT = 2
_split_streams = {}


def _split_stream(device, j=1):
    key = (device.type, device.index, j)
    if key not in _split_streams:
        _split_streams[key] = torch.cuda.Stream(device=device)
    return _split_streams[key]
```

### gm3d_amd/gemm.py

```python
import torch

from ._capi import lib
from .ops import _launch, _ptr, _stream


ENABLED = True
FUSE_GELU = True
FUSE_POOL = True
FUSE_GELU_BWD = True


def supported(x, w):
    return (ENABLED and x.is_cuda and x.dtype == torch.bfloat16 and w.dtype == torch.bfloat16 and x.dim() == 2 and w.dim() == 2
            and x.shape[1] == w.shape[1] and w.shape[0] % 128 == 0 and w.shape[1] % 64 == 0 and x.stride(1) == 1
            and w.stride(1) == 1 and x.stride(0) % 8 == 0 and w.stride(0) % 8 == 0 and x.stride(0) >= x.shape[1] and w.stride(0) >= w.shape[1]
            and x.data_ptr() % 16 == 0 and w.data_ptr() % 16 == 0)


RAGGED = True


def ragged_supported(x, w):
    return (ENABLED and RAGGED and x.is_cuda and x.dtype == torch.bfloat16 and w.dtype == torch.bfloat16 and x.dim() == 2 and w.dim() == 2
            and x.shape[1] == w.shape[1] and w.shape[0] % 8 == 0 and w.shape[1] % 8 == 0 and w.shape[1] >= 8 and x.stride(1) == 1
            and w.stride(1) == 1 and x.stride(0) % 8 == 0 and w.stride(0) % 8 == 0 and x.stride(0) >= x.shape[1] and w.stride(0) >= w.shape[1]
            and x.data_ptr() % 16 == 0 and w.data_ptr() % 16 == 0)


def linear_tn(x, w, bias=None, out=None):
    M, K = x.shape
    N = w.shape[0]
    if out is None:
        out = torch.empty(M, N, dtype=torch.bfloat16, device=x.device)
    _launch("gm3d_gemm_tn_bf16", {"M": M, "N": N, "K": K}, lib.gm3d_gemm_tn_bf16, _ptr(x), _ptr(w), _ptr(bias), _ptr(out), M, N, K,
            x.stride(0), w.stride(0), out.stride(0), _stream())
    return out


def linear_tn_ring(x, w, bias=None, out=None, bm=None):
    M, K = x.shape
    N = w.shape[0]
    if out is None:
        out = torch.empty(M, N, dtype=torch.bfloat16, device=x.device)
    if bm is None:
        bm = 64 if M <= 4096 else 128
    _launch("gm3d_gemm_tn_bf16_ring", {"M": M, "N": N, "K": K}, lib.gm3d_gemm_tn_bf16_ring, _ptr(x), _ptr(w), _ptr(bias), _ptr(out), M, N,
            K, x.stride(0), w.stride(0), out.stride(0), int(bm), _stream())
    return out


def linear_tn_ring96(x, w, bias=None, out=None, bm=64):
    M, K = x.shape
    N = w.shape[0]
    if out is None:
        out = torch.empty(M, N, dtype=torch.bfloat16, device=x.device)
    _launch("gm3d_gemm_tn_bf16_ring96", {"M": M, "N": N, "K": K}, lib.gm3d_gemm_tn_bf16_ring96, _ptr(x), _ptr(w), _ptr(bias), _ptr(out),
            M, N, K, x.stride(0), w.stride(0), out.stride(0), int(bm), _stream())
    return out


USE_DMA = True


def dma_bm(M):
    return 64 if M <= 4096 else 128


def dma_supported(x, w):
    return USE_DMA and supported(x, w) and w.shape[0] % 192 == 0 and x.data_ptr() % 16 == 0 and w.data_ptr() % 16 == 0


def linear_tn_dma(x, w, bias=None, out=None, bm=64):
    M, K = x.shape
    N = w.shape[0]
    if out is None:
        out = torch.empty(M, N, dtype=torch.bfloat16, device=x.device)
    _launch("gm3d_gemm_tn_bf16_dma", {"M": M, "N": N, "K": K}, lib.gm3d_gemm_tn_bf16_dma, _ptr(x), _ptr(w), _ptr(bias), _ptr(out), M, N,
            K, x.stride(0), w.stride(0), out.stride(0), int(bm), _stream())
    return out


def linear_gelu_dma(x, w, bias, f_out=None, g_out=None, bm=64):
    M, K = x.shape
    N = w.shape[0]
    if g_out is None:
        g_out = torch.empty(M, N, dtype=torch.bfloat16, device=x.device)
    _launch("gm3d_gemm_tn_bf16_dma_gelu", {"M": M, "N": N, "K": K}, lib.gm3d_gemm_tn_bf16_dma_gelu, _ptr(x), _ptr(w), _ptr(bias),
            _ptr(f_out), _ptr(g_out), M, N, K, x.stride(0), w.stride(0), f_out.stride(0) if f_out is not None else 0,
            g_out.stride(0), int(bm), _stream())
    return f_out, g_out


FUSE_LN = False


def linear_res(x, w, bias, res, rowscale, rows_per_sample, add, bm=None):
    M, K = x.shape
    N = w.shape[0]
    U = torch.empty(M, N, dtype=torch.float32, device=x.device)
    U16 = torch.empty(M, N, dtype=torch.bfloat16, device=x.device)
    stats = torch.empty(3, M, 2, dtype=torch.float32, device=x.device)
    if bm is None:
        bm = 64 if M <= 4096 else 128
    _launch("gm3d_gemm_tn_bf16_res", {"M": M, "N": N, "K": K}, lib.gm3d_gemm_tn_bf16_res, _ptr(x), _ptr(w), _ptr(bias), _ptr(res),
            _ptr(rowscale), int(rows_per_sample), _ptr(add), _ptr(U), _ptr(U16), _ptr(stats), M, N, K, x.stride(0), w.stride(0), int(bm),
            _stream())
    return U, U16, stats


def linear_lna(U, stats, gamma, beta, eps, w, bias=None, gelu=False, f_out=None, g_out=None, h_out=None, want_stats=False):
    M, K = U.shape
    N = w.shape[0]
    dev = U.device
    mean = torch.empty(M, dtype=torch.float32, device=dev) if want_stats else None
    rstd = torch.empty(M, dtype=torch.float32, device=dev) if want_stats else None
    if gelu:
        if g_out is None:
            g_out = torch.empty(M, N, dtype=torch.bfloat16, device=dev)
        _launch("gm3d_gemm_tn_bf16_lna", {"M": M, "N": N, "K": K}, lib.gm3d_gemm_tn_bf16_lna, _ptr(U), _ptr(stats), _ptr(gamma),
                _ptr(beta), float(eps), _ptr(w), _ptr(bias), _ptr(f_out), _ptr(g_out), _ptr(h_out), _ptr(mean), _ptr(rstd), M, N, K,
                U.stride(0), w.stride(0), f_out.stride(0) if f_out is not None else 0, g_out.stride(0), _stream())
        return f_out, g_out, mean, rstd
    c = torch.empty(M, N, dtype=torch.bfloat16, device=dev)
    _launch("gm3d_gemm_tn_bf16_lna", {"M": M, "N": N, "K": K}, lib.gm3d_gemm_tn_bf16_lna, _ptr(U), _ptr(stats), _ptr(gamma), _ptr(beta),
            float(eps), _ptr(w), _ptr(bias), _ptr(c), None, _ptr(h_out), _ptr(mean), _ptr(rstd), M, N, K, U.stride(0), w.stride(0),
            c.stride(0), 0, _stream())
    return c, mean, rstd


def linear_gelu(x, w, bias, f_out=None, g_out=None):
    M, K = x.shape
    N = w.shape[0]
    if g_out is None:
        g_out = torch.empty(M, N, dtype=torch.bfloat16, device=x.device)
    _launch("gm3d_gemm_tn_bf16_gelu", {"M": M, "N": N, "K": K}, lib.gm3d_gemm_tn_bf16_gelu, _ptr(x), _ptr(w), _ptr(bias),
            _ptr(f_out), _ptr(g_out), M, N, K, x.stride(0), w.stride(0), f_out.stride(0) if f_out is not None else 0,
            g_out.stride(0), _stream())
    return f_out, g_out


USE_WS = True
USE_WS_POOL = True


def ws_supported(x, w, pool=False):
    return ((USE_WS_POOL if pool else USE_WS) and supported(x, w) and x.shape[0] >= 32768
            and bool(lib.gm3d_gemm_ws_supported(w.shape[0], w.shape[1], int(pool))))


DMA192_BM64 = True
DMA192_RAGGED = True
WS_RAGGED = True


def ws_ragged_supported(x, w):
    return (USE_WS and WS_RAGGED and ragged_supported(x, w) and x.shape[0] >= 32768
            and (w.shape[0] % 128 != 0 or w.shape[1] % 64 != 0) and bool(lib.gm3d_gemm_ws_supported(w.shape[0], w.shape[1], 0)))


def linear_tn_ws(x, w, bias=None, out=None):
    M, K = x.shape
    N = w.shape[0]
    if out is None:
        out = torch.empty(M, N, dtype=torch.bfloat16, device=x.device)
    _launch("gm3d_gemm_tn_bf16_ws", {"M": M, "N": N, "K": K}, lib.gm3d_gemm_tn_bf16_ws, _ptr(x), _ptr(w), _ptr(bias), _ptr(out), M, N, K,
            x.stride(0), w.stride(0), out.stride(0), _stream())
    return out


WS_BN = True


WS_BN_STATS16 = False


def ws_bn_supported(x, w, t, group_rows=32):
    return (WS_BN and group_rows in (16, 32) and ws_supported(x, w) and x.shape[0] % 32 == 0 and t.dtype == torch.bfloat16 and t.is_contiguous()
            and t.shape == (x.shape[0] // group_rows, w.shape[0]) and lib.gm3d_gemm_ws_stats_rows(x.shape[0], w.shape[0], x.shape[1]) > 0)


def linear_ws_bn_apply(x, w, t, scale, shift, slope=0.0, group_rows=32):
    M, K = x.shape
    N = w.shape[0]
    out = torch.empty(M, N, dtype=torch.bfloat16, device=x.device)
    _launch("gm3d_gemm_tn_bf16_ws_bn_apply", {"M": M, "N": N, "K": K}, lib.gm3d_gemm_tn_bf16_ws_bn_apply_g, _ptr(x), _ptr(w), _ptr(t),
            _ptr(scale), _ptr(shift), float(slope), _ptr(out), M, N, K, x.stride(0), w.stride(0), t.stride(0), out.stride(0), int(group_rows),
            _stream())
    return out


def linear_ws_bn_stats(x, w, t, group_rows=32):
    M, K = x.shape
    N = w.shape[0]
    out = torch.empty(M, N, dtype=torch.bfloat16, device=x.device)
    rows = lib.gm3d_gemm_ws_stats_rows(M, N, K)
    part = torch.empty(rows, 2 * N, dtype=torch.float32, device=x.device)
    _launch("gm3d_gemm_tn_bf16_ws_bn_stats", {"M": M, "N": N, "K": K}, lib.gm3d_gemm_tn_bf16_ws_bn_stats_g, _ptr(x), _ptr(w), _ptr(t), _ptr(out),
            _ptr(part), M, N, K, x.stride(0), w.stride(0), t.stride(0), out.stride(0), int(group_rows), _stream())
    return out, part


def linear_tn_dmaw(x, w, bias=None, out=None, bm=128, bn=256):
    M, K = x.shape
    N = w.shape[0]
    if out is None:
        out = torch.empty(M, N, dtype=torch.bfloat16, device=x.device)
    _launch("gm3d_gemm_tn_bf16_dmaw", {"M": M, "N": N, "K": K}, lib.gm3d_gemm_tn_bf16_dmaw, _ptr(x), _ptr(w), _ptr(bias), _ptr(out), M,
            N, K, x.stride(0), w.stride(0), out.stride(0), int(bm), int(bn), _stream())
    return out


OWN_KT = (2, 4, 6, 8, 16, 18, 24)


def choose(M, N, K):
    if N == 384 and K in (384, 1024, 1152, 1536):
        return "ring64" if M <= 4096 else "ring128"
    if (N, K) == (1152, 384):
        return "ring128" if M <= 3200 else ("dma64x192" if M <= 4096 else "dma128x192") if USE_DMA else "own"
    if K == 384 and N % 192 == 0 and N > 384 and M < 32768:
        return ("dma64x192" if M <= 4096 else "dma128x192") if USE_DMA else "own"
    if M >= 32768:
        return "dma128x192" if N % 192 == 0 else "dma128x128"
    if (N, K) == (256, 512) or (N, K) == (128, 384):
        return "ring64"
    if N == 1024:
        return "dma128x128"
    return "dma64x128"


def mm(x, w, bias=None, out=None):
    how = choose(x.shape[0], w.shape[0], w.shape[1]) if supported(x, w) else "lib"
    if how == "lib" and ws_ragged_supported(x, w) and (out is None or (out.stride(1) == 1 and out.stride(0) % 8 == 0)):
        return linear_tn_ws(x, w, bias, out)
    if (how == "lib" and DMA192_RAGGED and USE_DMA and ragged_supported(x, w) and w.shape[0] % 192 == 0 and w.shape[1] % 64 == 0
            and x.shape[0] >= 8192 and (out is None or (out.stride(1) == 1 and out.stride(0) % 8 == 0))):
        tiles128 = -(-x.shape[0] // 128) * (w.shape[0] // 192)
        return linear_tn_dmaw(x, w, bias, out, bm=64 if (DMA192_BM64 and tiles128 < 512) else dma_bm(x.shape[0]), bn=192)
    if how == "lib" and ragged_supported(x, w) and (out is None or (out.stride(1) == 1 and out.stride(0) % 8 == 0)):
        if w.shape[1] % 64 == 0:
            return linear_tn_ring(x, w, bias, out)
        return linear_tn(x, w, bias, out)
    if how != "lib" and ws_supported(x, w):
        return linear_tn_ws(x, w, bias, out)
    if how == "own":
        return linear_tn(x, w, bias, out)
    if how.startswith("ring"):
        return linear_tn_ring(x, w, bias, out, bm=int(how[4:]))
    if how.startswith("dma"):
        bm, bn = how[3:].split("x")
        return linear_tn_dmaw(x, w, bias, out, bm=int(bm), bn=int(bn))
    y = x @ w.t()
    if bias is not None:
        y = y + bias.to(y.dtype)
    return y if out is None else out.copy_(y)


def transposed(w):
    N, K = w.shape
    if w.dtype == torch.bfloat16 and w.is_contiguous() and N % 8 == 0 and K % 8 == 0 and w.is_cuda and w.data_ptr() % 16 == 0:
        out = torch.empty(K, N, dtype=w.dtype, device=w.device)
        _launch("gm3d_transpose_bf16_batched", {"batch": 1, "rows": N, "cols": K}, lib.gm3d_transpose_bf16_batched, _ptr(w), _ptr(out),
                1, N, K, N * K, _stream())
        return out
    return w.t().contiguous()


_tr_known = {}
_tr_cache = None


def _tr_key(w):
    return (w.data_ptr(), tuple(w.shape))


def forget_transposes():
    _tr_known.clear()
    drop_transposes()


def prepare_transposes():
    global _tr_cache
    live = list(_tr_known.values())
    _tr_cache = {}
    for i in range(0, len(live), 8):
        chunk = live[i:i + 8]
        outs = stacked_transposes([[w] for w in chunk]) if len(chunk) > 1 else [transposed(chunk[0]).unsqueeze(0)]
        for w, o in zip(chunk, outs):
            _tr_cache[_tr_key(w)] = o[0]


def drop_transposes():
    global _tr_cache
    _tr_cache = None


def _transposed_for_mm_nn(w):
    if _tr_cache is not None:
        hit = _tr_cache.get(_tr_key(w))
        if hit is not None:
            return hit
        if (len(_tr_known) < 64 and w.is_contiguous() and w.dtype == torch.bfloat16 and w.shape[0] % 8 == 0 and w.shape[1] % 8 == 0
                and w.data_ptr() % 16 == 0 and not torch.cuda.is_current_stream_capturing()):
            _tr_known.setdefault(_tr_key(w), w)
    return transposed(w.contiguous())


def mm_nn(x, w, out=None):
    if (ENABLED and x.is_cuda and x.dtype == torch.bfloat16 and w.dtype == torch.bfloat16 and x.dim() == 2 and w.dim() == 2
            and w.shape[1] % 8 == 0 and w.shape[0] % 8 == 0 and x.stride(1) == 1 and x.stride(0) % 8 == 0 and x.data_ptr() % 16 == 0):
        wt = _transposed_for_mm_nn(w)
        if supported(x, wt) or ragged_supported(x, wt):
            return mm(x, wt, None, out)
    y = x @ w
    return y if out is None else out.copy_(y)


POOL_ON_DMA = True


def pool16_supported(x, w):
    N, K = w.shape
    return (USE_WS_POOL and ENABLED and x.is_cuda and x.dtype == torch.bfloat16 and w.dtype == torch.bfloat16 and x.dim() == 2
            and x.shape[0] >= 32768 and x.shape[0] % 16 == 0 and x.shape[1] == K and x.stride(1) == 1 and w.stride(1) == 1
            and x.stride(0) % 8 == 0 and w.stride(0) % 8 == 0 and x.data_ptr() % 16 == 0 and w.data_ptr() % 16 == 0
            and bool(lib.gm3d_gemm_ws_supported(N, K, 1)))


def linear_pool(x, w, bias, bias_after_pool, want_rows, group_rows=32):
    M, K = x.shape
    N = w.shape[0]
    rows = torch.empty(M, N, dtype=torch.bfloat16, device=x.device) if want_rows else None
    pooled = torch.empty(M // group_rows, N, dtype=torch.bfloat16, device=x.device)
    arg = torch.empty(M // group_rows, N, dtype=torch.uint8, device=x.device)
    if group_rows == 16:
        _launch("gm3d_gemm_tn_bf16_ws_pool", {"M": M, "N": N, "K": K}, lib.gm3d_gemm_tn_bf16_ws_poolg, _ptr(x), _ptr(w), _ptr(bias), _ptr(rows),
                _ptr(pooled), _ptr(arg), M, N, K, x.stride(0), w.stride(0), N, N, int(bias_after_pool), 16, _stream())
        return rows, pooled, arg
    if ws_supported(x, w, pool=True):
        _launch("gm3d_gemm_tn_bf16_ws_pool", {"M": M, "N": N, "K": K}, lib.gm3d_gemm_tn_bf16_ws_pool, _ptr(x), _ptr(w), _ptr(bias), _ptr(rows),
                _ptr(pooled), _ptr(arg), M, N, K, x.stride(0), w.stride(0), N, N, int(bias_after_pool), _stream())
        return rows, pooled, arg
    if POOL_ON_DMA and N % 8 == 0 and (N % 192 == 0 or N % 128 == 0):
        bn = 192 if N % 192 == 0 else 128
        _launch("gm3d_gemm_tn_bf16_dma_pool", {"M": M, "N": N, "K": K}, lib.gm3d_gemm_tn_bf16_dma_pool, _ptr(x), _ptr(w), _ptr(bias),
                _ptr(rows), _ptr(pooled), _ptr(arg), M, N, K, x.stride(0), w.stride(0), N, N, int(bias_after_pool), 128, bn, _stream())
        return rows, pooled, arg
    _launch("gm3d_gemm_tn_bf16_pool", {"M": M, "N": N, "K": K}, lib.gm3d_gemm_tn_bf16_pool, _ptr(x), _ptr(w), _ptr(bias), _ptr(rows),
            _ptr(pooled), _ptr(arg), M, N, K, x.stride(0), w.stride(0), N, N, int(bias_after_pool), _stream())
    return rows, pooled, arg


OWN_WGRAD = True


def wgrad_supported(dy, x):
    edge = 8 if RAGGED else 128
    return (ENABLED and OWN_WGRAD and dy.is_cuda and dy.dtype == torch.bfloat16 and x.dtype == torch.bfloat16 and dy.dim() == 3
            and x.dim() == 3 and dy.shape[:2] == x.shape[:2] and dy.shape[2] % edge == 0 and x.shape[2] % edge == 0
            and dy.shape[1] % 32 == 0 and dy.stride(2) == 1 and x.stride(2) == 1 and dy.stride(1) % 8 == 0 and x.stride(1) % 8 == 0
            and dy.stride(1) >= dy.shape[2] and x.stride(1) >= x.shape[2]
            and dy.data_ptr() % 16 == 0 and x.data_ptr() % 16 == 0 and (dy.shape[0] == 1 or (dy.stride(0) % 8 == 0 and x.stride(0) % 8 == 0)))


FUSE_SLAB_SUM = False
FUSE_SLAB_SUM_MAX = 8
_nt_counters = {}


def _nt_counter_slice(device, need):
    key = str(device)
    ent = _nt_counters.get(key)
    if ent is None:
        if device.type == "cuda" and torch.cuda.is_current_stream_capturing():
            return None
        ent = _nt_counters[key] = [torch.zeros(1 << 16, dtype=torch.int32, device=device), 0]
    buf, off = ent
    if need > buf.numel():
        return None
    if off + need > buf.numel():
        off = 0
    ent[1] = off + need
    return buf[off:off + need]


from . import streams as _streams_mod
_streams_mod.before_capture(lambda device: _nt_counter_slice(device, 0))


def wgrad_nt(dy, x, out=None, splits=None, big_tiles=False):
    nb, R, N = dy.shape
    K = x.shape[2]
    assert not big_tiles or splits is not None, "big_tiles: gm3d_gemm_nt_splits speaks for the 128 x 128 kernel, name the splits"
    name = "gm3d_gemm_nt_bf16_big" if big_tiles else "gm3d_gemm_nt_bf16"
    fn = getattr(lib, name)
    if splits is None:
        splits = lib.gm3d_gemm_nt_splits(nb, R, N, K)
    if out is None:
        out = torch.empty(nb, N, K, dtype=torch.float32, device=dy.device)
    assert out.dtype == torch.float32 and out.stride(2) == 1 and out.stride(1) >= K
    if splits == 1:
        _launch(name, {"B": nb, "M": R, "N": N, "K": K}, fn, _ptr(dy), _ptr(x), _ptr(out), nb, R, N, K,
                dy.stride(1), x.stride(1), out.stride(1), dy.stride(0), x.stride(0), out.stride(0), 1, 0, _stream())
        return out
    part = torch.empty(nb, splits, N, K, dtype=torch.float32, device=dy.device)
    if (FUSE_SLAB_SUM and not big_tiles and splits <= FUSE_SLAB_SUM_MAX and K % 4 == 0 and out.stride(1) % 4 == 0 and out.data_ptr() % 16 == 0
            and (nb == 1 or out.stride(0) >= N * out.stride(1))):
        cnt = _nt_counter_slice(dy.device, nb * lib.gm3d_gemm_nt_tiles(N, K))
        if cnt is not None:
            _launch("gm3d_gemm_nt_bf16_sum", {"B": nb, "M": R, "N": N, "K": K}, lib.gm3d_gemm_nt_bf16_sum, _ptr(dy), _ptr(x), _ptr(part),
                    _ptr(out), _ptr(cnt), nb, R, N, K, dy.stride(1), x.stride(1), out.stride(1), dy.stride(0), x.stride(0), out.stride(0),
                    splits, _stream())
            return out
    _launch(name, {"B": nb, "M": R, "N": N, "K": K}, fn, _ptr(dy), _ptr(x), _ptr(part), nb, R, N, K,
            dy.stride(1), x.stride(1), K, dy.stride(0), x.stride(0), splits * N * K, splits, N * K, _stream())
    if out.is_contiguous() or (out.stride(1) == K and out.stride(0) == N * K):
        _launch("gm3d_sum_few_rows", {"rows": nb * splits, "cols": N * K}, lib.gm3d_sum_few_rows, _ptr(part), nb, splits, N * K, _ptr(out),
                _stream())
    else:
        out.copy_(part.sum(dim=1))
    return out


MULTI_TARGET_WGS = 512
MULTI_SPLITS_MAX = 2
MULTI_WGRAD = True


def wgrad_multi_ok(dy, x, out):
    nb, R, N = dy.shape
    K = x.shape[2]
    return (wgrad_supported(dy, x) and K % 4 == 0
            and (out is None or (out.dtype == torch.float32 and out.shape == (nb, N, K) and out.stride(2) == 1 and out.stride(1) == K
                                 and (nb == 1 or out.stride(0) >= N * K) and out.data_ptr() % 16 == 0)))


def wgrad_nt_multi(reqs, splits=None, want_splits=False):
    import ctypes
    n = len(reqs)
    VP, I, LL = ctypes.c_void_p * n, ctypes.c_int * n, ctypes.c_longlong * n
    outs, parts, spl = [], [], []
    tiles = [r[0].shape[0] * ((r[0].shape[2] + 127) // 128) * ((r[1].shape[2] + 127) // 128) for r in reqs]
    tiles_all = sum(tiles)
    rows_target = max(512, sum(t_ * r[0].shape[1] for t_, r in zip(tiles, reqs)) // MULTI_TARGET_WGS)
    for dy, x, out in reqs:
        nb, R, N = dy.shape
        K = x.shape[2]
        if out is None:
            out = torch.empty(nb, N, K, dtype=torch.float32, device=dy.device)
        s_ = lib.gm3d_gemm_nt_splits(nb, R, N, K)
        if splits is not None:
            s_ = splits[len(spl)]
        elif MULTI_SPLITS_MAX and tiles_all < 768:
            s_ = 1
            while 2 * s_ <= min(64, R // rows_target) and R % (64 * s_) == 0:
                s_ *= 2
        elif MULTI_SPLITS_MAX and tiles_all >= 768:
            s_ = min(s_, MULTI_SPLITS_MAX if R > 4096 else 1)
            while s_ > 1 and R % (32 * s_):
                s_ -= 1
        outs.append(out)
        spl.append(s_)
        parts.append(torch.empty(nb, s_, N, K, dtype=torch.float32, device=dy.device) if s_ > 1 else None)
    _launch("gm3d_gemm_nt_bf16_multi", {"count": n, "problems": [(r[0].shape[0], r[0].shape[1], r[0].shape[2], r[1].shape[2]) for r in reqs],
                                        "splits": list(spl)}, lib.gm3d_gemm_nt_bf16_multi, n,
            VP(*[_ptr(r[0]) for r in reqs]), VP(*[_ptr(r[1]) for r in reqs]), VP(*[_ptr(o) for o in outs]),
            VP(*[(_ptr(p) if p is not None else None) for p in parts]), I(*[r[0].shape[0] for r in reqs]), I(*[r[0].shape[1] for r in reqs]),
            I(*[r[0].shape[2] for r in reqs]), I(*[r[1].shape[2] for r in reqs]), I(*[r[0].stride(1) for r in reqs]),
            I(*[r[1].stride(1) for r in reqs]), LL(*[r[0].stride(0) for r in reqs]), LL(*[r[1].stride(0) for r in reqs]),
            LL(*[o.stride(0) for o in outs]), I(*spl), _stream())
    return (outs, spl) if want_splits else outs


def tile_rows(M):
    return lib.gm3d_gemm_tile_rows(int(M))


def linear_gelu_bwd(d_o, w2t, f, bias, df, colpart):
    M, K = d_o.shape
    N = w2t.shape[0]
    _launch("gm3d_gemm_tn_bf16_gelu_bwd", {"M": M, "N": N, "K": K}, lib.gm3d_gemm_tn_bf16_gelu_bwd, _ptr(d_o), _ptr(w2t), _ptr(f),
            _ptr(bias), _ptr(df), _ptr(colpart), M, N, K, d_o.stride(0), w2t.stride(0), f.stride(0), df.stride(0), _stream())
    return df


def linear_gelu_bwd_dma(d_o, w2t, f, bias, df, colpart, bm=64):
    M, K = d_o.shape
    N = w2t.shape[0]
    assert colpart.shape[0] * bm >= M and colpart.shape[1] == N
    _launch("gm3d_gemm_tn_bf16_dma_gelu_bwd", {"M": M, "N": N, "K": K}, lib.gm3d_gemm_tn_bf16_dma_gelu_bwd, _ptr(d_o), _ptr(w2t),
            _ptr(f), _ptr(bias), _ptr(df), _ptr(colpart), M, N, K, d_o.stride(0), w2t.stride(0), f.stride(0), df.stride(0), int(bm),
            _stream())
    return df


MULTI_TRANSPOSE = True


def stacked_transposes(groups):
    import ctypes
    ok = MULTI_TRANSPOSE and 1 < len(groups) <= 8
    metas = []
    for ws in groups:
        w0 = ws[0]
        n = len(ws)
        step = (ws[1].data_ptr() - w0.data_ptr()) if n > 1 else w0.numel() * w0.element_size()
        regular = (w0.dtype == torch.bfloat16 and w0.is_cuda and w0.dim() == 2 and w0.shape[0] % 8 == 0 and w0.shape[1] % 8 == 0
                   and w0.data_ptr() % 16 == 0 and step % 16 == 0 and step > 0 and step % w0.element_size() == 0 and step // w0.element_size() >= w0.numel()
                   and all(w.shape == w0.shape and w.is_contiguous() and w.data_ptr() - w0.data_ptr() == i * step for i, w in enumerate(ws)))
        ok = ok and regular
        metas.append((w0, n, step // w0.element_size()))
    if not ok:
        return [stacked_transpose(ws) for ws in groups]
    outs = [torch.empty(n, w0.shape[1], w0.shape[0], dtype=w0.dtype, device=w0.device) for w0, n, _ in metas]
    c = len(groups)
    VP, I, LL = ctypes.c_void_p * c, ctypes.c_int * c, ctypes.c_longlong * c
    _launch("gm3d_transpose_bf16_multi", {"count": c}, lib.gm3d_transpose_bf16_multi, c, VP(*[_ptr(m_[0]) for m_ in metas]),
            VP(*[_ptr(o) for o in outs]), I(*[m_[1] for m_ in metas]), I(*[m_[0].shape[0] for m_ in metas]),
            I(*[m_[0].shape[1] for m_ in metas]), LL(*[m_[2] for m_ in metas]), _stream())
    return outs


def stacked_transpose(ws):
    w0 = ws[0]
    n = len(ws)
    if n > 1:
        step = ws[1].data_ptr() - w0.data_ptr()
        regular = step > 0 and step % w0.element_size() == 0 and all(
            w.shape == w0.shape and w.is_contiguous() and w.untyped_storage().data_ptr() == w0.untyped_storage().data_ptr()
            and w.data_ptr() - w0.data_ptr() == i * step for i, w in enumerate(ws))
        if (regular and w0.shape[0] % 8 == 0 and w0.shape[1] % 8 == 0 and w0.dtype == torch.bfloat16 and w0.data_ptr() % 16 == 0
                and step % 16 == 0):
            N, K = w0.shape
            out = torch.empty(n, K, N, dtype=w0.dtype, device=w0.device)
            _launch("gm3d_transpose_bf16_batched", {"batch": n, "rows": N, "cols": K}, lib.gm3d_transpose_bf16_batched, _ptr(w0),
                    _ptr(out), n, N, K, step // w0.element_size(), _stream())
            return out
        if regular:
            N, K = w0.shape
            v = torch.as_strided(w0, (n, N, K), (step // w0.element_size(), K, 1))
            return v.transpose(1, 2).contiguous()
    return torch.stack(list(ws)).transpose(1, 2).contiguous()
```

### gm3d_amd/masked_stack.py

```python
import torch

from ._capi import lib
from . import fused, gemm
from .embed import _c32
from .fused import PER_BLOCK, block_params, weight_cache
from .ops import _DT, _launch, _ptr, _stream


def _add_ln_fwd(x, y, ybias, rowscale, rps, z, gamma, beta, eps, adt, want_s, h_out=None):
    R, C = x.shape
    dev = x.device
    s = torch.empty(R, C, dtype=adt, device=dev) if want_s else None
    if gamma is None:
        _launch("gm3d_add_ln_fwd", {"R": R, "C": C, "dtype": str(adt)}, lib.gm3d_add_ln_fwd, _ptr(x), _ptr(y), _ptr(ybias), _ptr(rowscale),
                int(rps), _ptr(z), None, None, 0.0, _ptr(s), None, None, None, R, C, _DT[adt], _stream())
        return s, None, None, None
    h = h_out if h_out is not None else torch.empty(R, C, dtype=adt, device=dev)
    mean = torch.empty(R, dtype=torch.float32, device=dev)
    rstd = torch.empty(R, dtype=torch.float32, device=dev)
    _launch("gm3d_add_ln_fwd", {"R": R, "C": C, "dtype": str(adt)}, lib.gm3d_add_ln_fwd, _ptr(x), _ptr(y), _ptr(ybias), _ptr(rowscale),
            int(rps), _ptr(z), _ptr(gamma), _ptr(beta), float(eps), _ptr(s), _ptr(h), _ptr(mean), _ptr(rstd), R, C, _DT[adt], _stream())
    return s, h, mean, rstd


def _add_ln_bwd(dh, gin, x, mean, rstd, gamma, rowscale, rps, dy, partial, adt, acc=None, acc_mode=0):
    ref = dh if dh is not None else gin
    R, C = ref.shape
    dx = torch.empty(R, C, dtype=adt, device=ref.device)
    _launch("gm3d_add_ln_bwd", {"R": R, "C": C, "dtype": str(adt)}, lib.gm3d_add_ln_bwd_acc, _ptr(dh), _ptr(gin), _ptr(x), _ptr(mean),
            _ptr(rstd), _ptr(gamma), _ptr(rowscale), int(rps), _ptr(dx), _ptr(dy), _ptr(partial), 3, _ptr(acc), int(acc_mode), R, C,
            _DT[adt], _stream())
    return dx


def _attn_fwd(qkv, bits, B, T, H, hd, scale, out):
    if bits is None and hd == 64 and T <= 128:
        return fused._attention_fwd(qkv, B, T, H, scale, out=out)
    lse = torch.empty(B, H, T, dtype=torch.float32, device=qkv.device)
    _launch("gm3d_attention_masked_fwd", {"B": B, "T": T, "H": H, "HD": hd, "dtype": str(qkv.dtype)}, lib.gm3d_attention_masked_fwd,
            _ptr(qkv), _ptr(bits), _ptr(out), _ptr(lse), B, T, H, hd, float(scale), _DT[qkv.dtype], _stream())
    return out, lse


def _attn_bwd(qkv, a, da, lse, bits, B, T, H, hd, scale, dqkv):
    if bits is None and hd == 64 and T <= 128:
        return fused._attention_bwd(qkv, a, da, lse, B, T, H, scale, dqkv=dqkv)
    _launch("gm3d_attention_masked_bwd", {"B": B, "T": T, "H": H, "HD": hd, "dtype": str(qkv.dtype)}, lib.gm3d_attention_masked_bwd,
            _ptr(qkv), _ptr(bits), _ptr(a), _ptr(da), _ptr(lse), _ptr(dqkv), B, T, H, hd, float(scale), _DT[qkv.dtype], _stream())
    return dqkv


FUSE_GELU = True


def supported(x, blocks):
    C = x.shape[-1]
    H = blocks[0].attn.num_heads
    return (x.is_cuda and x.dim() == 3 and C % 8 == 0 and 8 <= C <= 512 and C % H == 0 and C // H in (16, 32, 64)
            and x.shape[1] <= 512 and x.dtype in (torch.float32, torch.bfloat16))


class MaskedStackFn(torch.autograd.Function):

    @staticmethod
    def forward(ctx, x, pos, bits, meta, *params):
        with torch.autocast("cuda", enabled=False):
            return MaskedStackFn._forward(ctx, x, pos, bits, meta, *params)

    @staticmethod
    def _forward(ctx, x, pos, bits, meta, *params):
        B, T, C = x.shape
        nblk = len(params) // PER_BLOCK
        adt, H, scale, eps = meta["adt"], meta["num_heads"], meta["scale"], meta["eps"]
        hd = C // H
        R = B * T
        dev = x.device
        s = x.reshape(R, C).to(adt).contiguous()
        posa = pos.reshape(R, C).to(adt).contiguous()
        need = meta["grad"] and any(ctx.needs_input_grad)
        if need:
            H1 = torch.empty(nblk, R, C, dtype=adt, device=dev)
            A = torch.empty(nblk, R, C, dtype=adt, device=dev)
            H2 = torch.empty(nblk, R, C, dtype=adt, device=dev)
            GG = torch.empty(nblk, R, 4 * C, dtype=adt, device=dev)
        y = yb = rs = None
        saved = []
        for i in range(nblk):
            ln1w, ln1b, wqkv, wproj, bproj, ln2w, ln2b, w1, b1, w2, b2 = params[i * PER_BLOCK:(i + 1) * PER_BLOCK]
            dp1, dp2 = meta["dp"][i]
            s1, h1, m1, r1 = _add_ln_fwd(s, y, yb, rs, T, posa, _c32(ln1w), _c32(ln1b), eps, adt, True, H1[i] if need else None)
            qkv = gemm.mm(h1, weight_cache.get(wqkv, adt))
            a, lse = _attn_fwd(qkv, bits, B, T, H, hd, scale, A[i] if need else torch.empty(R, C, dtype=adt, device=dev))
            p = gemm.mm(a, weight_cache.get(wproj, adt))
            s2, h2, m2, r2 = _add_ln_fwd(s1, p, _c32(bproj), dp1, T, None, _c32(ln2w), _c32(ln2b), eps, adt, True, H2[i] if need else None)
            W1 = weight_cache.get(w1, adt)
            if FUSE_GELU and adt == torch.bfloat16 and gemm.FUSE_GELU and gemm.dma_supported(h2, W1):
                f, g = gemm.linear_gelu_dma(h2, W1, _c32(b1), f_out=torch.empty(R, 4 * C, dtype=adt, device=dev) if need else None,
                                            g_out=GG[i] if need else None, bm=gemm.dma_bm(R))
            else:
                f = gemm.mm(h2, W1)
                g = fused.bias_gelu_fwd(f, _c32(b1), adt, g=GG[i] if need else None)
            y, yb, rs, s = gemm.mm(g, weight_cache.get(w2, adt)), _c32(b2), dp2, s2
            if need:
                saved += [s1, m1, r1, qkv, lse, s2, m2, r2, f]
        out, _, _, _ = _add_ln_fwd(s, y, yb, rs, T, None, None, None, 0.0, adt, True)
        if need:
            ctx.save_for_backward(H1, A, H2, GG, *params, *saved)
            ctx.bits = bits
        ctx.meta, ctx.shape, ctx.nblk, ctx.in_dtypes = meta, (B, T, C), nblk, (x.dtype, pos.dtype)
        return out.view(B, T, C)

    @staticmethod
    def backward(ctx, dout):
        with torch.autocast("cuda", enabled=False):
            return MaskedStackFn._backward(ctx, dout)

    @staticmethod
    def _backward(ctx, dout):
        meta, (B, T, C), nblk = ctx.meta, ctx.shape, ctx.nblk
        adt, H, scale = meta["adt"], meta["num_heads"], meta["scale"]
        hd, R = C // H, B * T
        bits = ctx.bits
        tens = ctx.saved_tensors
        H1, A, H2, GG = tens[:4]
        params = tens[4:4 + nblk * PER_BLOCK]
        saved = tens[4 + nblk * PER_BLOCK:]
        grads = [None] * (nblk * PER_BLOCK)
        dev = dout.device
        gin = dout.reshape(R, C).to(adt).contiguous()
        DO = torch.empty(nblk, R, C, dtype=adt, device=dev)
        DF = torch.empty(nblk, R, 4 * C, dtype=adt, device=dev)
        DP = torch.empty(nblk, R, C, dtype=adt, device=dev)
        DQ = torch.empty(nblk, R, 3 * C, dtype=adt, device=dev)
        PLN = torch.empty(2 * nblk + 1, lib.gm3d_ln_plain_partial_rows(R), 3 * C, dtype=torch.float32, device=dev)
        SLN = torch.empty(2 * nblk + 1, 3 * C, dtype=torch.float32, device=dev)
        W2T, WPT, W1T, WQT = gemm.stacked_transposes(
            [[weight_cache.get(params[i * PER_BLOCK + k], adt) for i in range(nblk)] for k in (9, 3, 7, 2)])
        dma_bwd = FUSE_GELU and adt == torch.bfloat16 and gemm.FUSE_GELU_BWD and gemm.dma_supported(gin, W2T[0])
        bm_bwd = gemm.dma_bm(R)
        PGL = torch.empty(nblk, (R + bm_bwd - 1) // bm_bwd if dma_bwd else lib.gm3d_gelu_partial_rows(R), 4 * C, dtype=torch.float32, device=dev)
        SGL = torch.empty(nblk, 4 * C, dtype=torch.float32, device=dev)
        G = _add_ln_bwd(None, gin, None, None, None, None, meta["dp"][nblk - 1][1], T, DO[nblk - 1], PLN[2 * nblk], adt)
        db2 = SLN[2 * nblk, 2 * C:]
        dpos = torch.empty(R, C, dtype=adt, device=dev)
        for i in range(nblk - 1, -1, -1):
            ln1w, ln1b, wqkv, wproj, bproj, ln2w, ln2b, w1, b1, w2, b2 = params[i * PER_BLOCK:(i + 1) * PER_BLOCK]
            s1, m1, r1, qkv, lse, s2, m2, r2, f = saved[i * 9:(i + 1) * 9]
            gi = grads[i * PER_BLOCK:(i + 1) * PER_BLOCK]
            gi[10] = db2
            if dma_bwd:
                gemm.linear_gelu_bwd_dma(DO[i], W2T[i], f, _c32(b1), DF[i], PGL[i], bm=bm_bwd)
            else:
                dg = gemm.mm(DO[i], W2T[i])
                fused.bias_gelu_bwd(dg, f, _c32(b1), adt, df=DF[i], partial=PGL[i])
            gi[8] = SGL[i]
            dh2 = gemm.mm(DF[i], W1T[i])
            G = _add_ln_bwd(dh2, G, s2, m2, r2, _c32(ln2w), meta["dp"][i][0], T, DP[i], PLN[2 * i + 1], adt)
            gi[5], gi[6], gi[4] = SLN[2 * i + 1, :C], SLN[2 * i + 1, C:2 * C], SLN[2 * i + 1, 2 * C:]
            da = gemm.mm(DP[i], WPT[i])
            _attn_bwd(qkv, A[i], da, lse, bits, B, T, H, hd, scale, DQ[i])
            dh1 = gemm.mm(DQ[i], WQT[i])
            G = _add_ln_bwd(dh1, G, s1, m1, r1, _c32(ln1w), meta["dp"][i - 1][1] if i > 0 else None, T, DO[i - 1] if i > 0 else None,
                            PLN[2 * i], adt, acc=dpos, acc_mode=1 if i == nblk - 1 else 2)
            gi[0], gi[1] = SLN[2 * i, :C], SLN[2 * i, C:2 * C]
            db2 = SLN[2 * i, 2 * C:]
            grads[i * PER_BLOCK:(i + 1) * PER_BLOCK] = gi
        fused.finish_batched(PLN, SLN)
        fused.finish_batched(PGL, SGL)
        from .optim import grad_slots

        def slot(k):
            ps = [params[i * PER_BLOCK + k] for i in range(nblk)]
            return grad_slots.stacked(ps) if dev.type == "cuda" and all(p.grad is None for p in ps) else None
        gw2, gw1, gwp, gwq = fused._wgrad_many([(DO, GG, slot(9)), (DF, H2, slot(7)), (DP, A, slot(3)), (DQ, H1, slot(2))])
        for i in range(nblk):
            grads[i * PER_BLOCK + 9], grads[i * PER_BLOCK + 7] = gw2[i], gw1[i]
            grads[i * PER_BLOCK + 3], grads[i * PER_BLOCK + 2] = gwp[i], gwq[i]
        for j, (gr, p) in enumerate(zip(grads, params)):
            if gr is not None and gr.dtype != p.dtype:
                grads[j] = gr.to(p.dtype)
        return (G.view(B, T, C).to(ctx.in_dtypes[0]), dpos.view(B, T, C).to(ctx.in_dtypes[1]), None, None) + tuple(grads)


def run_stack(blocks, x, pos, bits, training, adt):
    from . import models_mae_learn_loss as M
    blocks = list(blocks)
    B = x.shape[0]
    probs = []
    for b in blocks:
        p = b.drop_path.drop_prob if isinstance(b.drop_path, M.DropPath) else 0.0
        probs += [p, p]
    scales = M.drop_path_scales(B, probs, training, x.device)
    meta = {"num_heads": blocks[0].attn.num_heads, "scale": blocks[0].attn.scale, "eps": blocks[0].norm1.eps, "adt": adt,
            "dp": [(scales[2 * i], scales[2 * i + 1]) for i in range(len(blocks))], "grad": torch.is_grad_enabled()}
    params = []
    for b in blocks:
        params += block_params(b)
    return MaskedStackFn.apply(x, pos, bits, meta, *params)


_overflow = {}


def overflow_flag(device):
    device = torch.device(device)
    if device.type == "cuda" and device.index is None:
        device = torch.device("cuda", torch.cuda.current_device())
    key = str(device)
    if key not in _overflow:
        _overflow[key] = torch.zeros(1, dtype=torch.int32, device=device)
    return _overflow[key]


fused._streams.before_capture(overflow_flag)


def partition_visible(masked, Tc):
    B, T = masked.shape
    m = masked.contiguous()
    m = m.view(torch.uint8) if m.dtype == torch.bool else m.to(torch.uint8)
    dev = masked.device
    i32 = dict(dtype=torch.int32, device=dev)
    out = {"perm_c": torch.empty(B, Tc, **i32), "perm_v": torch.empty(B, Tc, **i32), "inv_v": torch.empty(B, T, **i32),
           "inv_m": torch.empty(B, T, **i32), "vis_c": torch.empty(B, Tc, dtype=torch.uint8, device=dev), "T": T, "Tc": Tc}
    _launch("gm3d_partition_visible", {"B": B, "T": T}, lib.gm3d_partition_visible, _ptr(m), B, T, Tc, _ptr(out["perm_c"]),
            _ptr(out["perm_v"]), _ptr(out["inv_v"]), _ptr(out["inv_m"]), _ptr(out["vis_c"]), _ptr(overflow_flag(dev)), _stream())
    return out


def select_rows(a, idx, alt=None):
    B, Ta, C = a.shape
    T = idx.shape[1]
    a = a.contiguous()
    if alt is not None:
        alt = alt.to(a.dtype).contiguous()
    out = torch.empty(B, T, C, dtype=a.dtype, device=a.device)
    _launch("gm3d_select_rows", {"B": B, "T": T, "C": C}, lib.gm3d_select_rows, _ptr(a), _ptr(idx), _ptr(alt), _ptr(out), B, Ta, T, C,
            a.element_size(), _stream())
    return out


class CompactFn(torch.autograd.Function):

    @staticmethod
    def forward(ctx, x, part):
        ctx.part = part
        return select_rows(x, part["perm_c"])

    @staticmethod
    def backward(ctx, dy):
        return select_rows(dy, ctx.part["inv_v"]), None


class MergeFn(torch.autograd.Function):

    @staticmethod
    def forward(ctx, y_c, tok, part):
        ctx.part = part
        ctx.dts = (y_c.dtype, tok.dtype)
        return select_rows(y_c, part["inv_v"], tok.to(y_c.dtype))

    @staticmethod
    def backward(ctx, dout):
        part = ctx.part
        d_yc = select_rows(dout, part["perm_v"])
        d_tok = select_rows(dout, part["inv_m"])
        return d_yc.to(ctx.dts[0]), d_tok.to(ctx.dts[1]), None
```

### include/gm3d.h

```cpp
#ifndef GM3D_H
#define GM3D_H
#include <stdint.h>

#ifdef __cplusplus
extern "C" {
#endif

typedef void *gm3d_stream_t;

enum {
    GM3D_OK = 0,
    GM3D_EINVAL = -1,
    GM3D_EUNSUPPORTED = -2,
    GM3D_ELAUNCH = -3
};

enum { GM3D_F32 = 0, GM3D_BF16 = 1 };

int gm3d_abi_version(void);
const char *gm3d_strerror(int code);

int gm3d_fps(const float *xyz, int B, int N, int npoint, int32_t *idx, float *centers,
             gm3d_stream_t stream);

int gm3d_gather_points(const float *feat, const int32_t *idx, int B, int C, int N, int M,
                       float *out, gm3d_stream_t stream);

int gm3d_gather_points_grad(const float *grad_out, const int32_t *idx, int B, int C, int N, int M,
                            float *grad_feat, gm3d_stream_t stream);

int gm3d_knn(const float *ref, const float *query, int B, int N, int G, int k,
             float *dist, int64_t *idx, gm3d_stream_t stream);

int gm3d_knn_group(const float *xyz, const float *center, int B, int N, int G, int k,
                   int64_t *idx, float *neighborhood, float *neighborhood_org,
                   gm3d_stream_t stream);

int gm3d_chamfer_fwd(const float *xyz1, const float *xyz2, int P, int n, int m,
                     float *dist1, float *dist2, int32_t *idx1, int32_t *idx2,
                     gm3d_stream_t stream);

int gm3d_chamfer_bwd(const float *xyz1, const float *xyz2, const int32_t *idx1, const int32_t *idx2,
                     const float *grad_dist1, const float *grad_dist2, int P, int n, int m,
                     float *gxyz1, float *gxyz2, gm3d_stream_t stream);

int gm3d_attention_fwd(const void *qkv, void *out, float *lse, int B, int T, int H,
                       float scale, int dtype, gm3d_stream_t stream);

int gm3d_attention_qkv_fwd(const void *h, const void *wqkv, void *out, float *lse, void *qkv_out,
                           int B, int T, int H, int C, float scale, int dtype, gm3d_stream_t stream);

int gm3d_attention_bwd(const void *qkv, const void *out, const void *dout, const float *lse,
                       void *dqkv, int B, int T, int H, float scale, int dtype,
                       gm3d_stream_t stream);

int gm3d_patch_chamfer_loss_fwd(const void *pred, long long pred_bstride, const float *target, const long long *ids,
                                long long ids_bstride, int B, int T, int M, float *matrix, int32_t *idx1, int32_t *idx2,
                                float *mean_out, int dtype, gm3d_stream_t stream);
int gm3d_patch_chamfer_loss_bwd(const void *pred, long long pred_bstride, const float *target, const long long *ids,
                                long long ids_bstride, const int32_t *idx1, const int32_t *idx2, const float *gmean, int B, int T,
                                int M, void *dpred, int dtype, gm3d_stream_t stream);
int gm3d_patch_chamfer_loss_bwd_full(const void *pred, long long pred_bstride, const float *target, const long long *ids,
                                     long long ids_bstride, const int32_t *idx1, const int32_t *idx2, const float *gmean, int B, int T,
                                     int M, int lead, void *dpred, int dtype, gm3d_stream_t stream);

int gm3d_ln_plain_partial_rows(int R);
int gm3d_ln_plain_fwd(const void *x, const float *gamma, const float *beta, float eps, void *h, float *mean, float *rstd, int R,
                      int C, int dtype, gm3d_stream_t stream);
int gm3d_ln_plain_bwd(const void *dh, const void *x, const float *mean, const float *rstd, const float *gamma, void *dx,
                      float *partial, int R, int C, int dtype, gm3d_stream_t stream);
int gm3d_add_ln_fwd(const void *x, const void *y, const float *ybias, const float *rowscale, int rows_per_sample, const void *z,
                    const float *gamma, const float *beta, float eps, void *s_out, void *h, float *mean, float *rstd, int R, int C,
                    int dtype, gm3d_stream_t stream);
int gm3d_add_ln_bwd(const void *dh, const void *gin, const void *x, const float *mean, const float *rstd, const float *gamma,
                    const float *rowscale, int rows_per_sample, void *dx, void *dy, float *partial, int nsum, int R, int C, int dtype,
                    gm3d_stream_t stream);
int gm3d_add_ln_bwd_acc(const void *dh, const void *gin, const void *x, const float *mean, const float *rstd, const float *gamma,
                        const float *rowscale, int rows_per_sample, void *dx, void *dy, float *partial, int nsum, void *acc,
                        int acc_mode, int R, int C, int dtype, gm3d_stream_t stream);


int gm3d_residual_ln_fwd(const float *res, const void *y, const float *bias, const float *rowscale,
                         int rows_per_sample, const void *add, const float *gamma, const float *beta,
                         float eps, float *out_res, void *h, float *mean, float *rstd, int R, int C,
                         int dtype, gm3d_stream_t stream);

int gm3d_residual_ln_bwd(const void *dh, const float *gin, const float *x, const float *mean,
                         const float *rstd, const float *gamma, const float *rowscale, int rows_per_sample,
                         float *dx, void *dy, float *acc, void *acc_out, float *partial, int R, int C, int dtype,
                         gm3d_stream_t stream);
int gm3d_ln_partial_rows(int R);

int gm3d_colsum_finish(const float *partial, int nrows, int pitch, int ncols, float *out, int accumulate,
                       gm3d_stream_t stream);

int gm3d_colsum_finish_batched(const float *partial, int njobs, long long job_stride, int nrows, int pitch, int ncols,
                               float *out, int out_stride, gm3d_stream_t stream);

int gm3d_bias_gelu_fwd(const void *f, const float *bias, void *g, int R, int C, int dtype,
                       gm3d_stream_t stream);
int gm3d_bias_gelu_bwd(const void *dg, const void *f, const float *bias, void *df, float *partial, int R,
                       int C, int dtype, gm3d_stream_t stream);
int gm3d_gelu_partial_rows(int R);

int gm3d_embed_partial_rows(int kind, int n, int C);

int gm3d_moments3(const float *x, int R, double *partial, gm3d_stream_t stream);

int gm3d_pn_layer1_fwd(const float *x, const float *wf, const float *bf, void *a1, int R, int C1, int dtype,
                       gm3d_stream_t stream);

int gm3d_group_max_fwd(const void *in, const float *bias, void *out, uint8_t *arg, int G, int K, int C, int dtype,
                       gm3d_stream_t stream);
int gm3d_group_max_bwd(const void *dout, const uint8_t *arg, void *din, int G, int K, int C, int dtype,
                       gm3d_stream_t stream);

int gm3d_bn_bcast_stats(const void *y0, const void *t, int G, int K, int C, float *partial, int dtype,
                        gm3d_stream_t stream);
int gm3d_bn_bcast_apply_relu(const void *y0, const void *t, const float *scale, const float *shift, void *a2,
                             int G, int K, int C, float slope, int dtype, gm3d_stream_t stream);
int gm3d_bn_bcast_bwd_stats(const void *da2, const void *y0, const void *t, const float *scale, const float *shift,
                            const float *mean, const float *rstd, int G, int K, int C, float *partial, float slope,
                            int dtype, gm3d_stream_t stream);
int gm3d_bn_bcast_bwd_apply(const void *da2, const void *y0, const void *t, const float *scale, const float *shift,
                            const float *mean, const float *rstd, const float *s1, const float *s2, void *dy,
                            float *dt, int G, int K, int C, float slope, int dtype, gm3d_stream_t stream);

int gm3d_head_fold(const float *W1, const float *b1, int nout, int C, float *wv, void *wv_t, float *bm, int dtype,
                   gm3d_stream_t stream);
int gm3d_head_rowdot(const void *a, const void *wv_t, const float *bm, int R, int C, float *out, int dtype, gm3d_stream_t stream);
int gm3d_head_fold_bwd(const float *dwv, const float *d, int R, int nout, int C, float *dW1, float *db1, gm3d_stream_t stream);
int gm3d_head_outer(const float *d, const float *wv, int R, int C, void *da, int dtype, gm3d_stream_t stream);

int gm3d_scale_translate(float *pc, const float *u, float lo, float span, float t, int B, int N, gm3d_stream_t stream);

int gm3d_group_select_maps(const long long *ids, int id_pitch, int B, int V, int G, int *sel, int *inv, gm3d_stream_t stream);
int gm3d_bn_bcast_apply_relu_sel(const void *y0, const void *t, const float *scale, const float *shift, void *a2,
                                 const int *sel, int G, int K, int C, float slope, int dtype, gm3d_stream_t stream);
int gm3d_bn_bcast_bwd_stats_sel(const void *da2, const void *y0, const void *t, const float *scale, const float *shift,
                                const float *mean, const float *rstd, const int *sel, int G, int K, int C, float *partial,
                                float slope, int dtype, gm3d_stream_t stream);
int gm3d_bn_bcast_bwd_apply_sel(const void *da2, const void *y0, const void *t, const float *scale, const float *shift,
                                const float *mean, const float *rstd, const float *s1, const float *s2, void *dy, float *dt,
                                const int *inv, int G, int K, int C, float slope, int dtype, gm3d_stream_t stream);

int gm3d_group_scatter_add(void *df, const void *dfg, const uint8_t *arg, int G, int K, int C, float *partial,
                           int dtype, gm3d_stream_t stream);

int gm3d_pn_layer1_bwd_stats(const void *da1, const void *a1, const float *x, const float *w1, const float *b1,
                             const float *mean, const float *rstd, const float *xmean, int R, int C1,
                             double *partial, int dtype, gm3d_stream_t stream);
int gm3d_colsum_finish_f64(const double *partial, int nrows, int pitch, int ncols, double *out,
                           gm3d_stream_t stream);

int gm3d_colsum_partial(const void *m, int R, int C, float *partial, int dtype, gm3d_stream_t stream);
int gm3d_colsum_partial_w(const void *m, const float *roww, int R, int C, float *partial, int dtype, gm3d_stream_t stream);

int gm3d_lin3_gelu_fwd(const float *x, const float *w, const float *b, void *out, int R, int C, int dtype,
                       gm3d_stream_t stream);
int gm3d_lin3_gelu_bwd(const void *dout, const float *x, const float *w, const float *b, int R, int C,
                       double *partial, int dtype, gm3d_stream_t stream);
int gm3d_lin3_finish(const double *partial, int nrows, int C, float *dW, float *db, gm3d_stream_t stream);

int gm3d_rank_loss(const float *pred, const float *target, int B, int M, float *out, float *dpred,
                   gm3d_stream_t stream);
int gm3d_rank_loss_tail(const float *pred, int ldp, const float *target, int B, int M, float *out, float *dpred, float *tot, float *loss,
                        gm3d_stream_t stream);
int gm3d_rank_loss_tail_bwd(const float *dpred, const float *g, const float *tot, int B, int M, int L, float *dfull, gm3d_stream_t stream);
int gm3d_ema_counters(long long *e, const long long *m, int n, float decay, float w, gm3d_stream_t stream);
int gm3d_drop_path_scales(const float *u, const float *keep, int S, int B, float *out, gm3d_stream_t stream);
int gm3d_pad_cols(const void *src, long long lds, int R, int N, void *dst, int Np, int dtype, gm3d_stream_t stream);

int gm3d_flat_partial_rows(long long n);
int gm3d_adamw_ema_flat_step(float *params, const float *grads, float *exp_avg, float *exp_avg_sq, float *ema,
                             void *shadow_p, void *shadow_e, long long n, long long n_decay, const float *lr_dev,
                             float weight_decay, float beta1, float beta2, float eps, const float *ema_w_dev,
                             float max_norm, float *step_dev, float *partial, float *scal, gm3d_stream_t stream);
int gm3d_adamw_ema_flat_step_lrd(float *params, const float *grads, float *exp_avg, float *exp_avg_sq, float *ema,
                                 void *shadow_p, void *shadow_e, long long n, long long n_decay, const float *lr_dev,
                                 const float *lr_scale, float weight_decay, float beta1, float beta2, float eps,
                                 const float *ema_w_dev, float max_norm, float *step_dev, float *partial, float *scal,
                                 gm3d_stream_t stream);

int gm3d_bn_finalize(const float *sums, double rows, const float *gamma, const float *beta, float eps, float momentum,
                     float *running_mean, float *running_var, long long *nbt, float *scale, float *shift,
                     float *mean_out, float *rstd_out, int C, int training, gm3d_stream_t stream);
int gm3d_pn1_finalize(const double *mom9, double rows, const float *w, const float *b, const float *gamma,
                      const float *beta, float eps, float momentum, float *running_mean, float *running_var,
                      long long *nbt, float *wf, float *bf, float *mean_out, float *rstd_out, double *mcov,
                      float *xmean, int C, int training, gm3d_stream_t stream);
int gm3d_pn1_bwd_finalize(const double *q, const double *mcov, const float *w, const float *gamma, const float *rstd,
                          float *dw, float *dgamma, float *dbeta, int C, gm3d_stream_t stream);
int gm3d_mask_select(const float *loss_pred, const float *noise, int B, int L, int len_keep, int len_loss, float *mask,
                     long long *vis_ids, long long *mask_ids, int id_pitch, gm3d_stream_t stream);
int gm3d_mask_select_b(const float *loss_pred, const float *noise, int B, int L, int len_keep, int len_loss, float *mask,
                       unsigned char *mask_bool, long long *vis_ids, long long *mask_ids, int id_pitch, gm3d_stream_t stream);
int gm3d_gemm_tn_bf16(const void *A, const void *W, const float *bias, void *C, int M, int N, int K, int lda, int ldw,
                      int ldc, gm3d_stream_t stream);
int gm3d_gemm_tn_bf16_gelu(const void *A, const void *W, const float *bias, void *F, void *G, int M, int N, int K, int lda,
                           int ldw, int ldf, int ldg, gm3d_stream_t stream);
int gm3d_gemm_tn_bf16_pool(const void *A, const void *W, const float *bias, void *C, void *P, uint8_t *arg, int M, int N, int K,
                           int lda, int ldw, int ldc, int ldp, int bias_after_pool, gm3d_stream_t stream);
int gm3d_gemm_tn_bf16_gelu_bwd(const void *dO, const void *Wt, const void *F, const float *bias, void *dF, float *colpart, int M,
                               int N, int K, int lda, int ldw, int ldf, int lddf, gm3d_stream_t stream);
int gm3d_gemm_tn_bf16_res(const void *A, const void *W, const float *bias, const float *res, const float *rowscale, int rows_per_sample,
                          const void *add, float *U, void *U16, float *stats, int M, int N, int K, int lda, int ldw, int bm,
                          gm3d_stream_t stream);
int gm3d_gemm_tn_bf16_lna(const void *U16, const float *stats, const float *gamma, const float *beta, float eps, const void *W,
                          const float *bias, void *C, void *G, void *H, float *mean, float *rstd, int M, int N, int K, int ldu, int ldw,
                          int ldc, int ldg, gm3d_stream_t stream);
int gm3d_gemm_tile_rows(int M);
int gm3d_gemm_tn_bf16_ring(const void *A, const void *W, const float *bias, void *C, int M, int N, int K, int lda, int ldw, int ldc,
                           int bm, gm3d_stream_t stream);
int gm3d_gemm_tn_bf16_ws(const void *A, const void *W, const float *bias, void *C, int M, int N, int K, int lda, int ldw, int ldc,
                         gm3d_stream_t stream);
int gm3d_gemm_tn_bf16_ws_pool(const void *A, const void *W, const float *bias, void *C, void *P, unsigned char *arg, int M, int N, int K,
                              int lda, int ldw, int ldc, int ldp, int bias_after_pool, gm3d_stream_t stream);
int gm3d_gemm_tn_bf16_ws_poolg(const void *A, const void *W, const float *bias, void *C, void *P, unsigned char *arg, int M, int N, int K,
                               int lda, int ldw, int ldc, int ldp, int bias_after_pool, int group_rows, gm3d_stream_t stream);
int gm3d_gemm_ws_supported(int N, int K, int pool);
int gm3d_gemm_tn_bf16_ws_bn_apply(const void *A, const void *W, const void *T, const float *scale, const float *shift, float slope, void *C,
                                  int M, int N, int K, int lda, int ldw, int ldt, int ldc, gm3d_stream_t stream);
int gm3d_gemm_tn_bf16_ws_bn_stats(const void *A, const void *W, const void *T, void *C, float *partial, int M, int N, int K, int lda,
                                  int ldw, int ldt, int ldc, gm3d_stream_t stream);
int gm3d_gemm_tn_bf16_ws_bn_apply_g(const void *A, const void *W, const void *T, const float *scale, const float *shift, float slope, void *C,
                                    int M, int N, int K, int lda, int ldw, int ldt, int ldc, int group_rows, gm3d_stream_t stream);
int gm3d_gemm_tn_bf16_ws_bn_stats_g(const void *A, const void *W, const void *T, void *C, float *partial, int M, int N, int K, int lda,
                                    int ldw, int ldt, int ldc, int group_rows, gm3d_stream_t stream);
int gm3d_gemm_ws_stats_rows(int M, int N, int K);
int gm3d_gemm_tn_bf16_ring96(const void *A, const void *W, const float *bias, void *C, int M, int N, int K, int lda, int ldw, int ldc,
                             int bm, gm3d_stream_t stream);
int gm3d_gemm_tn_bf16_dma(const void *A, const void *W, const float *bias, void *C, int M, int N, int K, int lda, int ldw, int ldc,
                          int bm, gm3d_stream_t stream);
int gm3d_gemm_tn_bf16_dmaw(const void *A, const void *W, const float *bias, void *C, int M, int N, int K, int lda, int ldw, int ldc,
                           int bm, int bn, gm3d_stream_t stream);
int gm3d_gemm_tn_bf16_dma_pool(const void *A, const void *W, const float *bias, void *C, void *P, unsigned char *arg, int M, int N,
                               int K, int lda, int ldw, int ldc, int ldp, int bias_after_pool, int bm, int bn, gm3d_stream_t stream);
int gm3d_gemm_tn_bf16_dma_gelu(const void *A, const void *W, const float *bias, void *F, void *G, int M, int N, int K, int lda,
                               int ldw, int ldf, int ldg, int bm, gm3d_stream_t stream);
int gm3d_gemm_tn_bf16_dma_gelu_bwd(const void *dO, const void *Wt, const void *F, const float *bias, void *dF, float *colpart, int M,
                                   int N, int K, int lda, int ldw, int ldf, int lddf, int bm, gm3d_stream_t stream);
int gm3d_transpose_bf16_batched(const void *src, void *dst, int batch, int rows, int cols, long long src_batch_stride,
                                gm3d_stream_t stream);
int gm3d_transpose_bf16_multi(int count, const void *const *src, void *const *dst, const int *batch, const int *rows, const int *cols,
                              const long long *src_batch_stride, gm3d_stream_t stream);
int gm3d_token_assemble_fwd(const void *tokens, const void *pos, const long long *order, int B, int L, int V, int C, void *x_vis,
                            void *pos_vis, void *pos_full, int dtype, gm3d_stream_t stream);
int gm3d_token_assemble_bwd(const void *dx_vis, const void *dpos_vis, const void *dpos_full, const long long *order, int B, int L,
                            int V, int C, void *dtokens, void *dpos, int dtype, gm3d_stream_t stream);
int gm3d_sum_few_rows(const float *partial, int njobs, int nrows, long long ncols, float *out, gm3d_stream_t stream);
int gm3d_gemm_nt_bf16(const void *dY, const void *X, float *out, int batch, int R, int N, int K, int ldy, int ldx, int ldo,
                      long long stride_y, long long stride_x, long long stride_o, int splits, long long stride_split,
                      gm3d_stream_t stream);
int gm3d_gemm_nt_splits(int batch, int R, int N, int K);
int gm3d_gemm_nt_bf16_big(const void *dY, const void *X, float *out, int batch, int R, int N, int K, int ldy, int ldx, int ldo,
                          long long stride_y, long long stride_x, long long stride_o, int splits, long long stride_split,
                          gm3d_stream_t stream);
int gm3d_gemm_nt_bf16_sum(const void *dY, const void *X, float *part, float *out, int *counters, int batch, int R, int N, int K, int ldy,
                          int ldx, int ldo, long long stride_y, long long stride_x, long long stride_o, int splits, gm3d_stream_t stream);
int gm3d_gemm_nt_tiles(int N, int K);
int gm3d_gemm_nt_bf16_multi(int count, const void *const *dY, const void *const *X, float *const *out, float *const *part, const int *batch,
                            const int *R, const int *N, const int *K, const int *ldy, const int *ldx, const long long *stride_y,
                            const long long *stride_x, const long long *stride_o, const int *splits, gm3d_stream_t stream);
int gm3d_gather_inverse(const long long *idx, int B, int J, int S, int *off, int *list, gm3d_stream_t stream);
int gm3d_gather_rows_bwd(const void *dy, const int *off, const int *list, void *dx, int B, int J, int S, int C, int dtype,
                         gm3d_stream_t stream);
int gm3d_radius_mask_bits(const float *center, const unsigned char *vis, float radius, int B, int G, unsigned *bits,
                          gm3d_stream_t stream);
int gm3d_radius_mask_bits_m(const float *center, const unsigned char *flags, int flags_are_masked, float radius, int B, int G,
                            unsigned *bits, gm3d_stream_t stream);
int gm3d_partition_visible(const unsigned char *masked, int B, int T, int Tc, int *perm_c, int *perm_v, int *inv_v, int *inv_m,
                           unsigned char *vis_c, int *overflow, gm3d_stream_t stream);
int gm3d_back_project(const unsigned char *masked_c, const long long *member, int B, int Gc, int k, int Gf, unsigned char *masked_f,
                      gm3d_stream_t stream);
int gm3d_interp3_fwd(const void *coarse, const long long *idx, const float *w, const void *fine, void *out, int B, int N, int S, int C1,
                     int C2, int dtype, gm3d_stream_t stream);
int gm3d_gather_rows_bwd_w(const void *dy, int ldy, int col0, int refs_per_row, const float *w, const int *off, const int *list, void *dx,
                           int B, int J, int S, int C, int dtype, gm3d_stream_t stream);
int gm3d_where_rows(const unsigned char *flag, int invert, const void *a, const void *alt, int alt_bcast, void *out, long long rows, int C,
                    int elem_bytes, gm3d_stream_t stream);
int gm3d_take_rows(const void *a, const long long *idx, void *out, int B, int S, int J, int C, int elem_bytes, gm3d_stream_t stream);
int gm3d_select_rows(const void *a, const int *idx, const void *alt, void *out, int B, int Ta, int T, int C, int elem_bytes,
                     gm3d_stream_t stream);
int gm3d_attention_masked_fwd(const void *qkv, const unsigned *mask, void *out, float *lse, int B, int T, int H, int HD, float scale,
                              int dtype, gm3d_stream_t stream);
int gm3d_attention_masked_bwd(const void *qkv, const unsigned *mask, const void *out, const void *dout, const float *lse, void *dqkv,
                              int B, int T, int H, int HD, float scale, int dtype, gm3d_stream_t stream);

int gm3d_vote_sample(const float *points, const int32_t *fps_idx, const long long *subsets, const float *scale, const float *shift,
                     int B, int N0, int point_all, int npoints, int V, float *out, gm3d_stream_t stream);
int gm3d_cls_tail_vote(const void *x, int V, int B, int T, int C, const float *W1, const float *b1, const float *g1, const float *be1,
                       const float *rm1, const float *rv1, const float *W2, const float *b2, const float *g2, const float *be2,
                       const float *rm2, const float *rv2, const float *W3, const float *b3, int cls_dim, float eps,
                       const long long *labels, float *mean, long long *pred, long long *correct, float *votes, int dtype,
                       gm3d_stream_t stream);

int gm3d_cls_tail_fwd(const void *x, int B, int T, int C, int mode, const float *W1, const float *b1, const float *g1, const float *be1,
                      const float *W2, const float *b2, const float *g2, const float *be2, const float *W3, const float *b3, int cls_dim,
                      float *rm1, float *rv1, long long *nbt1, float *rm2, float *rv2, long long *nbt2, float eps, float momentum,
                      int training, const float *drop, const long long *labels, float *feat, int *argmax, float *h, float *stats,
                      float *logits, float *loss, int dtype, gm3d_stream_t stream);
int gm3d_cls_tail_bwd(int B, int T, int C, int mode, const float *W1, const float *g1, const float *be1, const float *W2, const float *g2,
                      const float *be2, const float *W3, int cls_dim, int training, const float *drop, const long long *labels,
                      const float *feat, const int *argmax, const float *h, const float *stats, const float *logits,
                      const float *dlogits, const float *dloss, float *ws, void *dx, float *dW1, float *db1, float *dg1, float *dbe1,
                      float *dW2, float *db2, float *dg2, float *dbe2, float *dW3, float *db3, int dtype, gm3d_stream_t stream);

int gm3d_cls_tail_vote_pool(const void *x, int V, int B, int T, int C, int mode, const float *W1, const float *b1, const float *g1,
                            const float *be1, const float *rm1, const float *rv1, const float *W2, const float *b2, const float *g2,
                            const float *be2, const float *rm2, const float *rv2, const float *W3, const float *b3, int cls_dim,
                            float eps, const long long *labels, float *mean, long long *pred, long long *correct, float *votes,
                            float *feat, int dtype, gm3d_stream_t stream);

int gm3d_svm_gram(const float *X, int n, int d, double *K, gm3d_stream_t stream);
int gm3d_svm_smo(const double *K, int n, int ncls, const int *class_start, double C, double tol, long long max_iter, double *alpha,
                 double *rho, int *iters, int *capped, gm3d_stream_t stream);
int gm3d_svm_weights(const float *X, int n, int d, int ncls, const int *class_start, const double *alpha, double *w,
                     gm3d_stream_t stream);
int gm3d_svm_predict(const float *X, int m, int d, int ncls, const double *w, const double *rho, const long long *labels,
                     long long *pred, long long *correct, gm3d_stream_t stream);

#ifdef __cplusplus
}
#endif
#endif
```

Before: 17310.

## Read non-transposed weights directly in backward GEMMs via LDS transpose reads

Adds NN variants of the ring and DMA GEMM kernels that load the weight matrix in its natural K-by-N layout and transpose fragments on the fly with ds_read_tr16 LDS reads. The backward passes of the transformer and masked stacks use these variants instead of building stacked transposed weight copies every step. This removes the per-step weight transpose kernels and their memory traffic. In exchange the inner loop issues two transposing LDS reads per fragment where it used to issue one vector read, which may change LDS bank behaviour and MFMA feed rate.

```diff
diff --git a/gm3d_amd/_capi.py b/gm3d_amd/_capi.py
--- a/gm3d_amd/_capi.py
+++ b/gm3d_amd/_capi.py
@@ -89,6 +89,9 @@
     "gm3d_gemm_tn_bf16_dma": [_vp, _vp, _vp, _vp, _i, _i, _i, _i, _i, _i, _i, _vp],
     "gm3d_gemm_tn_bf16_dma_gelu_bwd": [_vp, _vp, _vp, _vp, _vp, _vp, _i, _i, _i, _i, _i, _i, _i, _i, _vp],
     "gm3d_gemm_tn_bf16_dma_gelu": [_vp, _vp, _vp, _vp, _vp, _i, _i, _i, _i, _i, _i, _i, _i, _vp],
+    "gm3d_gemm_tn_bf16_ring_nn": [_vp, _vp, _vp, _vp, _i, _i, _i, _i, _i, _i, _i, _vp],
+    "gm3d_gemm_tn_bf16_dmaw_nn": [_vp, _vp, _vp, _vp, _i, _i, _i, _i, _i, _i, _i, _i, _vp],
+    "gm3d_gemm_tn_bf16_dma_gelu_bwd_nn": [_vp, _vp, _vp, _vp, _vp, _vp, _i, _i, _i, _i, _i, _i, _i, _i, _vp],
     "gm3d_transpose_bf16_batched": [_vp, _vp, _i, _i, _i, ctypes.c_longlong, _vp],
     "gm3d_transpose_bf16_multi": [_i, _vp, _vp, _vp, _vp, _vp, _vp, _vp],
     "gm3d_token_assemble_fwd": [_vp, _vp, _vp, _i, _i, _i, _i, _vp, _vp, _vp, _i, _vp],
diff --git a/gm3d_amd/csrc/gemm_dma.hip b/gm3d_amd/csrc/gemm_dma.hip
--- a/gm3d_amd/csrc/gemm_dma.hip
+++ b/gm3d_amd/csrc/gemm_dma.hip
@@ -4,7 +4,7 @@
 
 constexpr int DBK = 64;
 
-template <int WMI, int EPI, int NJ>
+template <int WMI, int EPI, int NJ, bool WNN = false>
 __global__ __launch_bounds__(256, 2) void gemm_tn_dma_kernel(const bf16_t* __restrict__ A, const bf16_t* __restrict__ W,
                                                              const float* __restrict__ bias, bf16_t* __restrict__ C, int M, int N, int K,
                                                              int lda, int ldw, int ldc, int tiles_n, int total_tiles,
@@ -35,14 +35,20 @@
             src[i] = A + (size_t)am * lda + ((pslot ^ swz(row)) << 3);
         } else {
             const int row = 8 * (p - PA) + prow;
-            src[i] = W + (size_t)(n0 + row) * ldw + ((pslot ^ swz(row)) << 3);
-        }
-    }
+            if (WNN) {
+                const int kr = row & 63;
+                src[i] = W + (size_t)kr * ldw + n0 + 64 * (row >> 6) + ((pslot ^ swz(kr)) << 3);
+            } else {
+                src[i] = W + (size_t)(n0 + row) * ldw + ((pslot ^ swz(row)) << 3);
+            }
+        }
+    }
+    const size_t wstep = WNN ? (size_t)DBK * ldw : (size_t)DBK;
 #define GM3D_DMA_STAGE(ST)                                                                          \
     {                                                                                               \
         const unsigned base = lds0 + ((ST) & 1) * STAGE;                                            \
         _Pragma("unroll") for (int i = 0; i < PIECES; ++i)                                          \
-            glds16(src[i] + (size_t)(ST) * DBK, base + 1024 * (w + 4 * i));                         \
+            glds16(src[i] + (size_t)(ST) * (w + 4 * i < PA ? (size_t)DBK : wstep), base + 1024 * (w + 4 * i)); \
     }
     f32x16 acc[WMI][NJ];
 #pragma unroll
@@ -67,7 +73,8 @@
             for (int i = 0; i < WMI; ++i) fa[i] = *reinterpret_cast<const bf16x8*>(as + swz_off(wm + 32 * i + r, 2 * s + hh));
 #pragma unroll
             for (int j = 0; j < NJ; ++j) {
-                const bf16x8 fw = *reinterpret_cast<const bf16x8*>(ws + swz_off(wn + 32 * j + r, 2 * s + hh));
+                const bf16x8 fw = WNN ? swz_frag_tr(ws + ((wn + 32 * j) >> 6) * 8192, 16 * s, hh, ((wn + 32 * j) & 63) + (lane & 16), lane)
+                                      : *reinterpret_cast<const bf16x8*>(ws + swz_off(wn + 32 * j + r, 2 * s + hh));
 #pragma unroll
                 for (int i = 0; i < WMI; ++i) acc[i][j] = mfma_bf16(fw, fa[i], acc[i][j]);
             }
@@ -189,7 +196,7 @@
 
 static int dma_launch(const void* A, const void* W, const float* bias, void* C, void* G, int M, int N, int K, int lda, int ldw, int ldc,
                       int ldg, int bm, gm3d_stream_t stream, const void* Fpre = nullptr, int ldfp = 0, float* colpart = nullptr,
-                      int bn = 192, uint8_t* ARG = nullptr, int bias_after_pool = 0) {
+                      int bn = 192, uint8_t* ARG = nullptr, int bias_after_pool = 0, bool wnn = false) {
     using namespace gm3d;
     if (!A || !W || (!C && !G) || M < 0 || N < 1 || K < 1) return GM3D_EINVAL;
     if ((G || Fpre) && !bias && !ARG) return GM3D_EINVAL;
@@ -197,7 +204,8 @@
     if (Fpre && (!C || !colpart || G || ldfp % 8 || ldfp < N || ((size_t)Fpre & 15))) return GM3D_EINVAL;
     if (bn != 128 && bn != 192 && bn != 256) return GM3D_EUNSUPPORTED;
     if ((G || Fpre) && !ARG && bn != 192) return GM3D_EUNSUPPORTED;
-    if (N % bn || K % DBK || lda % 8 || ldw % 8 || lda < K || ldw < K || (C && (ldc % 8 || ldc < N)) || (G && (ldg % 8 || ldg < N)))
+    if (wnn && (G || ARG)) return GM3D_EUNSUPPORTED;
+    if (N % bn || K % DBK || lda % 8 || ldw % 8 || lda < K || ldw < (wnn ? N : K) || (C && (ldc % 8 || ldc < N)) || (G && (ldg % 8 || ldg < N)))
         return GM3D_EUNSUPPORTED;
     if ((((size_t)A | (size_t)W | (size_t)C | (size_t)G) & 15) || (bm != 64 && bm != 128)) return GM3D_EUNSUPPORTED;
     if (M == 0) return GM3D_OK;
@@ -209,6 +217,17 @@
     launch_lds<gemm_tn_dma_kernel<WMI, EPI, NJ>>(dim3(grid), dim3(256), lds, stream, (const bf16_t*)A, (const bf16_t*)W, bias,  \
                                                  (bf16_t*)C, M, N, K, lda, ldw, ldc, tiles_n, total, (bf16_t*)G, ldg,          \
                                                  (const bf16_t*)Fpre, ldfp, colpart, ARG, bias_after_pool)
+    if (wnn) {
+#define GM3D_DMA_NN(WMI, EPI, NJ)                                                                                                \
+    launch_lds<gemm_tn_dma_kernel<WMI, EPI, NJ, true>>(dim3(grid), dim3(256), lds, stream, (const bf16_t*)A, (const bf16_t*)W, bias,  \
+                                                       (bf16_t*)C, M, N, K, lda, ldw, ldc, tiles_n, total, (bf16_t*)G, ldg,          \
+                                                       (const bf16_t*)Fpre, ldfp, colpart, ARG, bias_after_pool)
+        if (Fpre) return bm == 64 ? GM3D_DMA_NN(1, 2, 3) : GM3D_DMA_NN(2, 2, 3);
+        if (bn == 192) return bm == 64 ? GM3D_DMA_NN(1, 0, 3) : GM3D_DMA_NN(2, 0, 3);
+        if (bn == 128) return bm == 64 ? GM3D_DMA_NN(1, 0, 2) : GM3D_DMA_NN(2, 0, 2);
+        return bm == 64 ? GM3D_DMA_NN(1, 0, 4) : GM3D_DMA_NN(2, 0, 4);
+#undef GM3D_DMA_NN
+    }
     if (ARG) {
         if (bn == 128) return bm == 64 ? GM3D_DMA(1, 3, 2) : GM3D_DMA(2, 3, 2);
         return bm == 64 ? GM3D_DMA(1, 3, 3) : GM3D_DMA(2, 3, 3);
@@ -251,3 +270,15 @@
     if (!F || !bias || !dF || !colpart) return GM3D_EINVAL;
     return dma_launch(dO, Wt, bias, dF, nullptr, M, N, K, lda, ldw, lddf, 0, bm, stream, F, ldf, colpart);
 }
+
+extern "C" int gm3d_gemm_tn_bf16_dmaw_nn(const void* A, const void* W, const float* bias, void* C, int M, int N, int K, int lda, int ldw,
+                                         int ldc, int bm, int bn, gm3d_stream_t stream) {
+    if (!C) return GM3D_EINVAL;
+    return dma_launch(A, W, bias, C, nullptr, M, N, K, lda, ldw, ldc, 0, bm, stream, nullptr, 0, nullptr, bn, nullptr, 0, true);
+}
+
+extern "C" int gm3d_gemm_tn_bf16_dma_gelu_bwd_nn(const void* dO, const void* W2, const void* F, const float* bias, void* dF, float* colpart,
+                                                 int M, int N, int K, int lda, int ldw, int ldf, int lddf, int bm, gm3d_stream_t stream) {
+    if (!F || !bias || !dF || !colpart) return GM3D_EINVAL;
+    return dma_launch(dO, W2, bias, dF, nullptr, M, N, K, lda, ldw, lddf, 0, bm, stream, F, ldf, colpart, 192, nullptr, 0, true);
+}
diff --git a/gm3d_amd/csrc/gemm_ring.hip b/gm3d_amd/csrc/gemm_ring.hip
--- a/gm3d_amd/csrc/gemm_ring.hip
+++ b/gm3d_amd/csrc/gemm_ring.hip
@@ -4,7 +4,7 @@
 
 constexpr int RBN = 128, RBK = 64, RNBUF = 4, RCP = 132;
 
-template <int WMI, bool RES, int DEPTH>
+template <int WMI, bool RES, int DEPTH, bool WNN = false>
 __global__ __launch_bounds__(256) void gemm_tn_ring_kernel(const bf16_t* __restrict__ A, const bf16_t* __restrict__ W,
                                                            const float* __restrict__ bias, bf16_t* __restrict__ C, int M, int N, int K,
                                                            int lda, int ldw, int ldc, int tiles_n, int total_tiles,
@@ -35,16 +35,23 @@
             src[i] = A + (size_t)am * lda + ((pslot ^ swz(row)) << 3);
         } else {
             const int row = 8 * (p - PA) + prow;
-            const int wn_ = n0 + row < N ? n0 + row : N - 1;
-            src[i] = W + (size_t)wn_ * ldw + ((pslot ^ swz(row)) << 3);
-        }
-    }
+            if (WNN) {
+                const int kr = row & 63;
+                const int col = n0 + 64 * (row >> 6) + ((pslot ^ swz(kr)) << 3);
+                src[i] = W + (size_t)kr * ldw + (col < N ? col : N - 8);
+            } else {
+                const int wn_ = n0 + row < N ? n0 + row : N - 1;
+                src[i] = W + (size_t)wn_ * ldw + ((pslot ^ swz(row)) << 3);
+            }
+        }
+    }
+    const size_t wstep = WNN ? (size_t)RBK * ldw : (size_t)RBK;
     constexpr int NBUF = DEPTH + 2;
 #define GM3D_RING_STAGE(ST)                                                                          \
     {                                                                                                \
         const unsigned base = lds0 + ((ST) % NBUF) * STAGE;                                          \
         _Pragma("unroll") for (int i = 0; i < PIECES; ++i)                                           \
-            glds16(src[i] + (size_t)(ST) * RBK, base + 1024 * (w + 4 * i));                          \
+            glds16(src[i] + (size_t)(ST) * (w + 4 * i < PA ? (size_t)RBK : wstep), base + 1024 * (w + 4 * i)); \
     }
 
     f32x16 acc[WMI][2];
@@ -79,7 +86,9 @@
 #pragma unroll
             for (int i = 0; i < WMI; ++i) fa[s][i] = *reinterpret_cast<const bf16x8*>(as + swz_off(wm + 32 * i + r, 2 * s + hh));
 #pragma unroll
-            for (int j = 0; j < 2; ++j) fw[s][j] = *reinterpret_cast<const bf16x8*>(ws + swz_off(wn + 32 * j + r, 2 * s + hh));
+            for (int j = 0; j < 2; ++j)
+                fw[s][j] = WNN ? swz_frag_tr(ws + (wn >> 6) * 8192, 16 * s, hh, 32 * j + (lane & 16), lane)
+                               : *reinterpret_cast<const bf16x8*>(ws + swz_off(wn + 32 * j + r, 2 * s + hh));
         }
 #pragma unroll
         for (int s = 0; s < 4; ++s)
@@ -275,11 +284,12 @@
 
 static int ring_launch(const void* A, const void* W, const float* bias, void* C, int M, int N, int K, int lda, int ldw, int ldc, int bm,
                        gm3d_stream_t stream, const float* res, const float* rowscale, int rows_per_sample, const void* add, float* U,
-                       float* stats, void* U16) {
+                       float* stats, void* U16, bool wnn = false) {
     using namespace gm3d;
     if (!A || !W || (!C && !U) || M < 0 || N < 1 || K < 1) return GM3D_EINVAL;
-    if (N % 8 || (U && N % RBN) || K % RBK || lda % 8 || ldw % 8 || lda < K || ldw < K || (C && (ldc % 8 || ldc < N)))
+    if (N % 8 || (U && N % RBN) || K % RBK || lda % 8 || ldw % 8 || lda < K || ldw < (wnn ? N : K) || (C && (ldc % 8 || ldc < N)))
         return GM3D_EUNSUPPORTED;
+    if (wnn && U) return GM3D_EUNSUPPORTED;
     if ((((size_t)A | (size_t)W) & 15) || (bm != 64 && bm != 128)) return GM3D_EUNSUPPORTED;
     if (M == 0) return GM3D_OK;
     const int tiles_m = (M + bm - 1) / bm, tiles_n = (N + RBN - 1) / RBN;
@@ -291,14 +301,27 @@
                                                           bias, (bf16_t*)C, M, N, K, lda, ldw, ldc, tiles_n, total, res, rowscale, \
                                                           rows_per_sample, (const bf16_t*)add, U, stats, (bf16_t*)U16)
     if (U) return bm == 64 ? GM3D_RING(1, true) : GM3D_RING(2, true);
-    return bm == 64 ? GM3D_RING(1, false) : GM3D_RING(2, false);
+    if (!wnn) return bm == 64 ? GM3D_RING(1, false) : GM3D_RING(2, false);
 #undef GM3D_RING
+    if (bm == 64)
+        return launch_lds<gemm_tn_ring_kernel<1, false, RING_DEPTH, true>>(dim3(grid), dim3(256), lds, stream, (const bf16_t*)A, (const bf16_t*)W,
+                                                                           bias, (bf16_t*)C, M, N, K, lda, ldw, ldc, tiles_n, total, res, rowscale,
+                                                                           rows_per_sample, (const bf16_t*)add, U, stats, (bf16_t*)U16);
+    return launch_lds<gemm_tn_ring_kernel<2, false, RING_DEPTH, true>>(dim3(grid), dim3(256), lds, stream, (const bf16_t*)A, (const bf16_t*)W, bias,
+                                                                       (bf16_t*)C, M, N, K, lda, ldw, ldc, tiles_n, total, res, rowscale,
+                                                                       rows_per_sample, (const bf16_t*)add, U, stats, (bf16_t*)U16);
 }
 
 extern "C" int gm3d_gemm_tn_bf16_ring(const void* A, const void* W, const float* bias, void* C, int M, int N, int K, int lda, int ldw,
                                       int ldc, int bm, gm3d_stream_t stream) {
     if (!C) return GM3D_EINVAL;
     return ring_launch(A, W, bias, C, M, N, K, lda, ldw, ldc, bm, stream, nullptr, nullptr, 1, nullptr, nullptr, nullptr, nullptr);
+}
+
+extern "C" int gm3d_gemm_tn_bf16_ring_nn(const void* A, const void* W, const float* bias, void* C, int M, int N, int K, int lda, int ldw,
+                                         int ldc, int bm, gm3d_stream_t stream) {
+    if (!C) return GM3D_EINVAL;
+    return ring_launch(A, W, bias, C, M, N, K, lda, ldw, ldc, bm, stream, nullptr, nullptr, 1, nullptr, nullptr, nullptr, nullptr, true);
 }
 
 extern "C" int gm3d_gemm_tn_bf16_ring96(const void* A, const void* W, const float* bias, void* C, int M, int N, int K, int lda, int ldw,
diff --git a/gm3d_amd/csrc/mfma.hpp b/gm3d_amd/csrc/mfma.hpp
--- a/gm3d_amd/csrc/mfma.hpp
+++ b/gm3d_amd/csrc/mfma.hpp
@@ -36,6 +36,18 @@
 __device__ __forceinline__ int swz(int row) { return (((row >> 1) & 1) << 2) | (((row >> 2) & 1) << 1) | ((row >> 3) & 1); }
 __device__ __forceinline__ int swz_off(int row, int ch) { return row * 128 + ((ch ^ swz(row)) << 4); }
 
+__device__ __forceinline__ bf16x8 swz_frag_tr(const unsigned char* img, int kk0, int hh, int colblk, int lane) {
+    const int l16 = lane & 15, q = l16 >> 2, p = l16 & 3;
+    const int col = colblk + 4 * p, ch = col >> 3, sub = ((col >> 2) & 1) << 3;
+    const int r0 = kk0 + 8 * hh + q, r1 = r0 + 4;
+    const bf16x4 lo = __builtin_amdgcn_ds_read_tr16_b64_v4bf16((lds_bf16x4*)(img + swz_off(r0, ch) + sub));
+    const bf16x4 hi = __builtin_amdgcn_ds_read_tr16_b64_v4bf16((lds_bf16x4*)(img + swz_off(r1, ch) + sub));
+    bf16x8 v;
+#pragma unroll
+    for (int j = 0; j < 4; ++j) { v[j] = lo[j]; v[4 + j] = hi[j]; }
+    return v;
+}
+
 __device__ __forceinline__ unsigned lds_addr(const unsigned char* p) {
     return (unsigned)(size_t)(__attribute__((address_space(3))) const unsigned char*)p;
 }
diff --git a/gm3d_amd/fused.py b/gm3d_amd/fused.py
--- a/gm3d_amd/fused.py
+++ b/gm3d_amd/fused.py
@@ -477,10 +477,13 @@
         SLN = torch.empty(2 * nblk + 1, 3, C, dtype=torch.float32, device=dev)
         w2s = [weight_cache.get(params[i * PER_BLOCK + 9], adt) for i in range(nblk)]
         fuse_mlp_bwd = gemm.ENABLED and gemm.FUSE_GELU_BWD and adt == torch.bfloat16 and dh.is_cuda
+        direct = False
         if fuse_mlp_bwd:
-            W2T, WPT, W1T, WQT = gemm.stacked_transposes(
-                [w2s] + [[weight_cache.get(params[i * PER_BLOCK + k], adt) for i in range(nblk)] for k in (3, 7, 2)])
-        dma_bwd = fuse_mlp_bwd and gemm.dma_supported(dh.reshape(R, C), W2T[0])
+            wps, w1s, wqs = [[weight_cache.get(params[i * PER_BLOCK + k], adt) for i in range(nblk)] for k in (3, 7, 2)]
+            direct = gemm.gelu_bwd_nn_supported(R, w2s[0]) and all(gemm.nn_how(R, w_) is not None for ws_ in (wps, w1s, wqs) for w_ in ws_)
+            if not direct:
+                W2T, WPT, W1T, WQT = gemm.stacked_transposes([w2s, wps, w1s, wqs])
+        dma_bwd = direct or (fuse_mlp_bwd and gemm.dma_supported(dh.reshape(R, C), W2T[0]))
         bm_bwd = gemm.dma_bm(R)
         PGL = torch.empty(nblk, ((R + bm_bwd - 1) // bm_bwd if dma_bwd else gemm.tile_rows(R)) if fuse_mlp_bwd
                           else lib.gm3d_gelu_partial_rows(R), 4 * C, dtype=torch.float32, device=dev)
@@ -497,20 +500,22 @@
             dp2_prev = meta["dp"][i - 1][1] if i > 0 else None
             gi = grads[i * PER_BLOCK:(i + 1) * PER_BLOCK]
             gi[10] = db2
-            if fuse_mlp_bwd:
+            if direct:
+                df = gemm.linear_gelu_bwd_dma_nn(d_o, w2s[i], f, b1, DF[i], PGL[i], bm=bm_bwd)
+            elif fuse_mlp_bwd:
                 df = (gemm.linear_gelu_bwd_dma(d_o, W2T[i], f, b1, DF[i], PGL[i], bm=bm_bwd) if dma_bwd
                       else gemm.linear_gelu_bwd(d_o, W2T[i], f, b1, DF[i], PGL[i]))
             else:
                 dg = d_o @ weight_cache.get(w2, adt)
                 df, _ = bias_gelu_bwd(dg, f, b1, adt, df=DF[i], partial=PGL[i])
             gi[8] = SGL[i]
-            dh2 = gemm.mm(df, W1T[i]) if fuse_mlp_bwd else df @ weight_cache.get(w1, adt)
+            dh2 = gemm.mm_nn(df, w1s[i]) if direct else gemm.mm(df, W1T[i]) if fuse_mlp_bwd else df @ weight_cache.get(w1, adt)
             dx1, d_p, _ = residual_ln_bwd(dh2, G, x1, m2, r2, ln2w, dp1, T, None, True, adt, R, dy=DP[i],
                                           partial=PLN[2 * i + 1])
             gi[5], gi[6], gi[4] = SLN[2 * i + 1, 0], SLN[2 * i + 1, 1], SLN[2 * i + 1, 2]
-            da = gemm.mm(d_p, WPT[i]) if fuse_mlp_bwd else d_p @ weight_cache.get(wproj, adt)
+            da = gemm.mm_nn(d_p, wps[i]) if direct else gemm.mm(d_p, WPT[i]) if fuse_mlp_bwd else d_p @ weight_cache.get(wproj, adt)
             dqkv = _attention_bwd(qkv, A[i], da, lse, B, T, H, scale, dqkv=DQ[i])
-            dh1 = gemm.mm(dqkv, WQT[i]) if fuse_mlp_bwd else dqkv @ weight_cache.get(wqkv, adt)
+            dh1 = gemm.mm_nn(dqkv, wqs[i]) if direct else gemm.mm(dqkv, WQT[i]) if fuse_mlp_bwd else dqkv @ weight_cache.get(wqkv, adt)
             last = DIRECT_INPUT_GRADS and i == 0 and nblk > 1 and adt != torch.float32 and ctx.in_dtypes == (adt, adt)
             if last:
                 dx_a = torch.empty(R, C, dtype=adt, device=dev)
diff --git a/gm3d_amd/gemm.py b/gm3d_amd/gemm.py
--- a/gm3d_amd/gemm.py
+++ b/gm3d_amd/gemm.py
@@ -306,7 +306,71 @@
     return transposed(w.contiguous())
 
 
+NN_DIRECT = True
+
+
+def nn_how(M, w, x=None, out=None):
+    if not (ENABLED and NN_DIRECT and w.is_cuda and w.dtype == torch.bfloat16 and w.dim() == 2):
+        return None
+    K, N = w.shape
+    if (K % 64 or N % 8 or w.stride(1) != 1 or w.stride(0) % 8 or w.stride(0) < N or w.data_ptr() % 16):
+        return None
+    if x is not None and not (x.is_cuda and x.dtype == torch.bfloat16 and x.dim() == 2 and x.shape == (M, K) and x.stride(1) == 1
+                              and x.stride(0) % 8 == 0 and x.stride(0) >= K and x.data_ptr() % 16 == 0):
+        return None
+    if out is not None and not (out.dtype == torch.bfloat16 and out.shape == (M, N) and out.stride(1) == 1 and out.stride(0) % 8 == 0
+                                and out.stride(0) >= N and out.data_ptr() % 16 == 0):
+        return None
+    if USE_WS and M >= 32768 and bool(lib.gm3d_gemm_ws_supported(N, K, 0)):
+        return None
+    if N % 128 == 0:
+        how = choose(M, N, K)
+        if how.startswith("ring"):
+            return ("ring", int(how[4:]))
+        if how.startswith("dma"):
+            bm, bn = how[3:].split("x")
+            return ("dma", int(bm), int(bn))
+        return None
+    if DMA192_RAGGED and USE_DMA and RAGGED and N % 192 == 0 and M >= 8192:
+        tiles128 = -(-M // 128) * (N // 192)
+        return ("dma", 64 if (DMA192_BM64 and tiles128 < 512) else dma_bm(M), 192)
+    return ("ring", 64 if M <= 4096 else 128) if RAGGED else None
+
+
+def linear_nn(x, w, how, out=None):
+    M, K = x.shape
+    N = w.shape[1]
+    if out is None:
+        out = torch.empty(M, N, dtype=torch.bfloat16, device=x.device)
+    if how[0] == "ring":
+        _launch("gm3d_gemm_tn_bf16_ring_nn", {"M": M, "N": N, "K": K}, lib.gm3d_gemm_tn_bf16_ring_nn, _ptr(x), _ptr(w), None, _ptr(out), M,
+                N, K, x.stride(0), w.stride(0), out.stride(0), how[1], _stream())
+    else:
+        _launch("gm3d_gemm_tn_bf16_dmaw_nn", {"M": M, "N": N, "K": K}, lib.gm3d_gemm_tn_bf16_dmaw_nn, _ptr(x), _ptr(w), None, _ptr(out), M,
+                N, K, x.stride(0), w.stride(0), out.stride(0), how[1], how[2], _stream())
+    return out
+
+
+def gelu_bwd_nn_supported(M, w2):
+    return (ENABLED and NN_DIRECT and USE_DMA and w2.is_cuda and w2.dtype == torch.bfloat16 and w2.dim() == 2 and w2.shape[0] % 64 == 0
+            and w2.shape[1] % 192 == 0 and w2.shape[1] % 128 == 0 and w2.stride(1) == 1 and w2.stride(0) % 8 == 0
+            and w2.stride(0) >= w2.shape[1] and w2.data_ptr() % 16 == 0)
+
+
+def linear_gelu_bwd_dma_nn(d_o, w2, f, bias, df, colpart, bm=64):
+    M, K = d_o.shape
+    N = w2.shape[1]
+    assert colpart.shape[0] * bm >= M and colpart.shape[1] == N and w2.shape[0] == K
+    _launch("gm3d_gemm_tn_bf16_dma_gelu_bwd_nn", {"M": M, "N": N, "K": K}, lib.gm3d_gemm_tn_bf16_dma_gelu_bwd_nn, _ptr(d_o), _ptr(w2),
+            _ptr(f), _ptr(bias), _ptr(df), _ptr(colpart), M, N, K, d_o.stride(0), w2.stride(0), f.stride(0), df.stride(0), int(bm),
+            _stream())
+    return df
+
+
 def mm_nn(x, w, out=None):
+    how = nn_how(x.shape[0], w, x, out) if x.dim() == 2 and w.dim() == 2 and x.shape[1] == w.shape[0] else None
+    if how is not None:
+        return linear_nn(x, w, how, out)
     if (ENABLED and x.is_cuda and x.dtype == torch.bfloat16 and w.dtype == torch.bfloat16 and x.dim() == 2 and w.dim() == 2
             and w.shape[1] % 8 == 0 and w.shape[0] % 8 == 0 and x.stride(1) == 1 and x.stride(0) % 8 == 0 and x.data_ptr() % 16 == 0):
         wt = _transposed_for_mm_nn(w)
diff --git a/gm3d_amd/masked_stack.py b/gm3d_amd/masked_stack.py
--- a/gm3d_amd/masked_stack.py
+++ b/gm3d_amd/masked_stack.py
@@ -134,9 +134,12 @@
         DQ = torch.empty(nblk, R, 3 * C, dtype=adt, device=dev)
         PLN = torch.empty(2 * nblk + 1, lib.gm3d_ln_plain_partial_rows(R), 3 * C, dtype=torch.float32, device=dev)
         SLN = torch.empty(2 * nblk + 1, 3 * C, dtype=torch.float32, device=dev)
-        W2T, WPT, W1T, WQT = gemm.stacked_transposes(
-            [[weight_cache.get(params[i * PER_BLOCK + k], adt) for i in range(nblk)] for k in (9, 3, 7, 2)])
-        dma_bwd = FUSE_GELU and adt == torch.bfloat16 and gemm.FUSE_GELU_BWD and gemm.dma_supported(gin, W2T[0])
+        w2s, wps, w1s, wqs = [[weight_cache.get(params[i * PER_BLOCK + k], adt) for i in range(nblk)] for k in (9, 3, 7, 2)]
+        direct = (FUSE_GELU and adt == torch.bfloat16 and gemm.FUSE_GELU_BWD and gemm.gelu_bwd_nn_supported(R, w2s[0])
+                  and all(gemm.nn_how(R, w_) is not None for ws_ in (wps, w1s, wqs) for w_ in ws_))
+        if not direct:
+            W2T, WPT, W1T, WQT = gemm.stacked_transposes([w2s, wps, w1s, wqs])
+        dma_bwd = direct or (FUSE_GELU and adt == torch.bfloat16 and gemm.FUSE_GELU_BWD and gemm.dma_supported(gin, W2T[0]))
         bm_bwd = gemm.dma_bm(R)
         PGL = torch.empty(nblk, (R + bm_bwd - 1) // bm_bwd if dma_bwd else lib.gm3d_gelu_partial_rows(R), 4 * C, dtype=torch.float32, device=dev)
         SGL = torch.empty(nblk, 4 * C, dtype=torch.float32, device=dev)
@@ -148,18 +151,20 @@
             s1, m1, r1, qkv, lse, s2, m2, r2, f = saved[i * 9:(i + 1) * 9]
             gi = grads[i * PER_BLOCK:(i + 1) * PER_BLOCK]
             gi[10] = db2
-            if dma_bwd:
+            if direct:
+                gemm.linear_gelu_bwd_dma_nn(DO[i], w2s[i], f, _c32(b1), DF[i], PGL[i], bm=bm_bwd)
+            elif dma_bwd:
                 gemm.linear_gelu_bwd_dma(DO[i], W2T[i], f, _c32(b1), DF[i], PGL[i], bm=bm_bwd)
             else:
                 dg = gemm.mm(DO[i], W2T[i])
                 fused.bias_gelu_bwd(dg, f, _c32(b1), adt, df=DF[i], partial=PGL[i])
             gi[8] = SGL[i]
-            dh2 = gemm.mm(DF[i], W1T[i])
+            dh2 = gemm.mm_nn(DF[i], w1s[i]) if direct else gemm.mm(DF[i], W1T[i])
             G = _add_ln_bwd(dh2, G, s2, m2, r2, _c32(ln2w), meta["dp"][i][0], T, DP[i], PLN[2 * i + 1], adt)
             gi[5], gi[6], gi[4] = SLN[2 * i + 1, :C], SLN[2 * i + 1, C:2 * C], SLN[2 * i + 1, 2 * C:]
-            da = gemm.mm(DP[i], WPT[i])
+            da = gemm.mm_nn(DP[i], wps[i]) if direct else gemm.mm(DP[i], WPT[i])
             _attn_bwd(qkv, A[i], da, lse, bits, B, T, H, hd, scale, DQ[i])
-            dh1 = gemm.mm(DQ[i], WQT[i])
+            dh1 = gemm.mm_nn(DQ[i], wqs[i]) if direct else gemm.mm(DQ[i], WQT[i])
             G = _add_ln_bwd(dh1, G, s1, m1, r1, _c32(ln1w), meta["dp"][i - 1][1] if i > 0 else None, T, DO[i - 1] if i > 0 else None,
                             PLN[2 * i], adt, acc=dpos, acc_mode=1 if i == nblk - 1 else 2)
             gi[0], gi[1] = SLN[2 * i, :C], SLN[2 * i, C:2 * C]
diff --git a/include/gm3d.h b/include/gm3d.h
--- a/include/gm3d.h
+++ b/include/gm3d.h
@@ -240,6 +240,12 @@
                                int ldw, int ldf, int ldg, int bm, gm3d_stream_t stream);
 int gm3d_gemm_tn_bf16_dma_gelu_bwd(const void *dO, const void *Wt, const void *F, const float *bias, void *dF, float *colpart, int M,
                                    int N, int K, int lda, int ldw, int ldf, int lddf, int bm, gm3d_stream_t stream);
+int gm3d_gemm_tn_bf16_ring_nn(const void *A, const void *W, const float *bias, void *C, int M, int N, int K, int lda, int ldw, int ldc,
+                              int bm, gm3d_stream_t stream);
+int gm3d_gemm_tn_bf16_dmaw_nn(const void *A, const void *W, const float *bias, void *C, int M, int N, int K, int lda, int ldw, int ldc,
+                              int bm, int bn, gm3d_stream_t stream);
+int gm3d_gemm_tn_bf16_dma_gelu_bwd_nn(const void *dO, const void *W2, const void *F, const float *bias, void *dF, float *colpart, int M,
+                                      int N, int K, int lda, int ldw, int ldf, int lddf, int bm, gm3d_stream_t stream);
 int gm3d_transpose_bf16_batched(const void *src, void *dst, int batch, int rows, int cols, long long src_batch_stride,
                                 gm3d_stream_t stream);
 int gm3d_transpose_bf16_multi(int count, const void *const *src, void *const *dst, const int *batch, const int *rows, const int *cols,
```

New measurement: 17380 (median of 6 runs). About the same (+0.4%).
